# taleinat/fuzzysearch

Hardware: AMD Instinct MI355X
Metric: GB/s of sequence scanned at |p|=20 max_l_dist=2 (levenshtein_ngram path; two searches in flight: see value_sync for one synchronous call at a time) (higher is better)
Workload: dtype u8

## Files before the change

fuzzysearch_amd/_native.py:

```python
import ctypes
import os
import threading

_HERE = os.path.dirname(os.path.abspath(__file__))
LIB_PATH = os.environ.get("FUZZYSEARCH_HIP_LIB") or os.path.join(_HERE, "libfzhip.so")

FZ_OK, FZ_EINVAL, FZ_ENOMEM, FZ_EDEVICE, FZ_EUNSUPPORTED, FZ_EHALO, FZ_ETIMEOUT = 0, -1, -2, -3, -4, -5, -6
UINT64_MAX = (1 << 64) - 1


class FzMatch(ctypes.Structure):
    _fields_ = [("start", ctypes.c_int64), ("end", ctypes.c_int64),
                ("dist", ctypes.c_int32), ("block", ctypes.c_int32)]


class FzRecordsInfo(ctypes.Structure):
    _fields_ = [("n_lines", ctypes.c_uint64), ("n_seqs", ctypes.c_uint64), ("packed_bytes", ctypes.c_uint64),
                ("bad_record", ctypes.c_uint64), ("bad_reason", ctypes.c_uint32)]


class FzDeriveInfo(ctypes.Structure):
    _fields_ = [("n_out", ctypes.c_uint64), ("packed_bytes", ctypes.c_uint64), ("longest", ctypes.c_uint64),
                ("bad_item", ctypes.c_uint64), ("bad_reason", ctypes.c_uint32)]

# ... 60 lines not shown
    "fz_search_end": _END,
    "fz_subs_ngrams": _SEARCH,
    "fz_generic_ngrams": _GENERIC,
    "fz_generic_ngrams_consolidated": _GENERIC,
    "fz_lev_ngrams_consolidated": _SEARCH,
    "fz_subs_ngrams_best": _SEARCH,
    "fz_lev_ngrams_multi": _MULTI,
    "fz_lev_ngrams_multi_consolidated": _MULTI,
    "fz_debug_multi_plan": (ci, (bp, u64p, u32, u32, u32p, u32p)),
    "fz_subs_ngrams_multi": _MULTI,
    "fz_subs_ngrams_multi_best": _MULTI,
    "fz_debug_multi_plan_mode": (ci, (u32, bp, u64p, u32, u32, u32p, u32p)),
    "fz_batch_upload": (ci, (vp, bp, u64p, u64, vpp)),
    "fz_batch_search": (ci, (vp, vp, u32, bp, u32, u32, ci, mpp, u32pp, u64p)),
    "fz_batch_search_multi": (ci, (vp, vp, u32, bp, u64p, u32, u32, ci, mpp, u32pp, u64pp)),
    "fz_batch_assign": (ci, (vp, vp, u32, bp, u64p, u32, u32, vpp)),
    "fz_debug_assign_fold": (ci, (vp, u64, vp, u64, u32, vp, u32, vp, u32, u32, vp)),
    "fz_batch_end_overlaps": (ci, (vp, vp, u32, bp, u64p, u32, u32, u32, vpp)),
    "fz_debug_end_overlaps": (ci, (u32, bp, u64p, u32, u32, u32, bp, vp, u64, vp)),
    "fz_debug_overlap_ms": (ci, (vp, f64p)),
    "fz_batch_score_cuts": (ci, (vp, vp, vp, vp, u32, u32, u32, vpp)),
    "fz_debug_score_cuts": (ci, (vp, vp, u32, u32, u32, bp, vp, u64, vp)),
    "fz_debug_cuts_ms": (ci, (vp, f64p)),
    "fz_subs_ngrams_multi_cls": _MULTI_CLS,
    "fz_subs_ngrams_multi_best_cls": _MULTI_CLS,
    "fz_batch_search_multi_cls": (ci, (vp, vp, bp, u64p, u32, u32, bp, bp, ci, mpp, u32pp, u64pp)),
    "fz_batch_assign_cls": (ci, (vp, vp, bp, u64p, u32, u32, bp, bp, vpp)),
    "fz_debug_multi_plan_cls": (ci, (bp, u64p, u32, u32, bp, bp, u32p, u32p, u32p, u32p)),
    "fz_debug_batch_segment": (ci, (u64p, u64, u64, u64p, u64p, u64p)),
    "fz_batch_upload_records": (ci, (vp, bp, u64, u32, u32, u32, vpp, rip)),
    "fz_batch_tables": (ci, (vp, vp, vp)),
    "fz_debug_batch_bytes": (ci, (vp, vp, u64)),
    "fz_debug_records_split": (ci, (bp, u64, u32, u32, u32, vpp, vpp, vpp, rip)),
    "fz_debug_scan_items": (u32, ()),
    "fz_debug_records_ms": (ci, (vp, f64p)),
    "fz_batch_upload_fasta": (ci, (vp, bp, u64, u32, vpp, rip)),
    "fz_batch_fasta_index": (ci, (vp, vp)),
    "fz_debug_fasta_split": (ci, (bp, u64, u32, vpp, vpp, vpp, rip)),
    "fz_debug_fasta_upper4": (u32, (u32,)),
    "fz_debug_fasta_src": (u64, (u64, u64, u64, u64)),
    "fz_batch_derive": (ci, (vp, vp, vp, vp, vp, u64, u32, bp, vpp, dip)),
    "fz_debug_derive_plan": (ci, (vp, u64, vp, vp, vp, u64, vp, vp, dip)),
    "fz_debug_derive_ms": (ci, (vp, f64p)),
    "fz_batch_upload_records_lines": (ci, (vp, bp, u64, u32, vp, u32, u32, vpp, rip)),
    "fz_batch_format": (ci, (vp, vp, u32, bp, vp, u32, u32, vp, u64, fip)),
    "fz_debug_format_plan": (ci, (vp, u32, u64, vp, u32, u32, vp, fip)),
    "fz_debug_format_ms": (ci, (vp, f64p)),
    "fz_subs_ngrams_any": _ANY,
    "fz_subs_lp_any": _ANY,
    "fz_generic_ngrams_any": (ci, (vp, vp, bp, u32, u32, u32, u32, u32, cip)),
    "fz_lev_lp": _SEARCH,
    "fz_subs_lp": _SEARCH,
    "fz_generic_lp": _GENERIC,
    "fz_comm_unique_id": (ci, (vp, u64)),
    "fz_comm_init_rank": (ci, (vp, vp, ci, ci)),
    "fz_comm_init_all": (ci, (vp,)),
    "fz_comm_info": (ci, (vp, cip, cip, cip)),
    "fz_comm_set_collective": (ci, (vp, ci)),
    "fz_comm_allgather": (ci, (vp, vp, u64, vp)),
    "fz_comm_max_f64": (ci, (vp, f64p)),
    "fz_comm_barrier": (ci, (vp,)),
    "fz_comm_destroy": (None, (vp,)),
    "fz_comm_gather_ms": (ci, (vp, f64p)),
    "fz_comm_backend": (ci, ()),
    "fz_consolidate": _REDUCE,
    "fz_group_best": _REDUCE,
    "fz_merge_ranks": (ci, (vp, vp, vp, u32, u32, vp)),
    "fz_wire_pack": (ci, (vp, u64, u64, vp)),
    "fz_wire_merge": (ci, (vp, u32, u64, u64, vp, u64, u64p, u64p)),
    "fz_stream_open": (ci, (vp, u32, bp, u32, u32, u32, u32, u32, u64, u32, u32, u64, vpp)),
    "fz_stream_buffer": (ci, (vp, vpp, u64p)),
    "fz_stream_submit": (ci, (vp, u64, ci)),
    "fz_stream_read_fd": (ci, (vp, ci, i64, ci, u64p)),
    "fz_stream_finish": (ci, (vp, mpp, u32pp, u64p)),
    "fz_stream_close": (None, (vp,)),
    "fz_debug_reload_switches": (None, ()),
    "fz_debug_launch_plan": (ci, (bp, u32, u32, u32p, u32, u32p)),
    "fz_debug_order_records": (ci, (vp, u64, u32, mpp, u64p)),
    "fz_debug_order_records_bounded": (ci, (vp, u64, u32, u64, u32, mpp, u64p)),
    "fz_debug_order_segments": (ci, (vp, vp, u32, u32, mpp, u64p)),
    "fz_debug_scan_regions": (ci, (u64, u64, u32, ci, f64, ci, u32p, vp)),
    "fz_debug_scan_plan": (ci, (cs, u32, u32, u64, u32, ci, u32p, u32p, cip, u32p, vp)),
    "fz_debug_scan_instance": (ci, (u32, cs, u32, u32, u64, u32, u32p, u32p, u32p)),
    "fz_debug_gather_merge": (ci, (vp, u32, u64, vp, u32, mpp, u64p, u64p)),
    "fz_stats": (ci, (vp, stp)),
    "fz_mem_info": (ci, (vp, u64p, u64p)),
    "fz_set_timing": (ci, (vp, ci)),
    "fz_set_streams": (ci, (vp, ci)),
    "fz_device_ms": (ci, (vp, f64p, ci)),
    "fz_free": (None, (vp,)),
}
EXPORTED_SYMBOLS = tuple(PROTOTYPES)

OPTIONAL = frozenset((
    "fz_batch_search_multi", "fz_batch_assign", "fz_debug_assign_fold",
    "fz_batch_end_overlaps", "fz_debug_end_overlaps", "fz_debug_overlap_ms",
    "fz_batch_score_cuts", "fz_debug_score_cuts", "fz_debug_cuts_ms",
    "fz_subs_ngrams_multi_cls", "fz_subs_ngrams_multi_best_cls", "fz_batch_search_multi_cls", "fz_batch_assign_cls",
    "fz_debug_multi_plan_cls",
    "fz_batch_upload_records", "fz_batch_tables", "fz_debug_batch_bytes", "fz_debug_records_split", "fz_debug_scan_items",
    "fz_debug_records_ms",
    "fz_batch_upload_fasta", "fz_batch_fasta_index", "fz_debug_fasta_split", "fz_debug_fasta_upper4", "fz_debug_fasta_src",
    "fz_batch_derive", "fz_debug_derive_plan", "fz_debug_derive_ms",
    "fz_batch_upload_records_lines", "fz_batch_format", "fz_debug_format_plan", "fz_debug_format_ms",
    "fz_debug_scan_plan", "fz_mem_info", "fz_debug_scan_instance",
))

_lib = None
_lib_lock = threading.Lock()


def load_library():
    global _lib
    with _lib_lock:
        if _lib is not None:
            return _lib
        if not os.path.exists(LIB_PATH):
            raise HipEngineError(
                "fuzzysearch_amd: %s is missing. Build it with `python -m fuzzysearch_amd.build` "
                "(hipcc, --offload-arch=gfx950). There is no CPU fallback." % LIB_PATH)
        L = ctypes.CDLL(LIB_PATH)
        for name, (restype, argtypes) in PROTOTYPES.items():
            if name in OPTIONAL and not hasattr(L, name):
                continue
            fn = getattr(L, name)
            fn.restype, fn.argtypes = restype, argtypes
        if L.fz_abi_version() != 1:
            raise HipEngineError("libfzhip.so ABI version mismatch")
        _lib = L
        return L


class UnsupportedSearch(NotImplementedError):
    """The search is outside what the GPU engine supports: a subsequence of more than 65 535 items, a Levenshtein
    budget above 1 023, a generic search (separate limits) or a linear-programming route with max_l_dist above 255,
    more than 255 distinct symbols in a subsequence that is neither bytes nor latin-1 text, automaton candidate sets
    beyond 2^18 entries.  Nothing was searched and there is no CPU fallback: a caller that needs such a search
    catches this and routes it to the reference implementation."""


def _entry(lib, name):
    fn = getattr(lib, name, None)
    if fn is None:
        raise UnsupportedSearch("this libfzhip.so has no %s: it was built before that entry point existed" % name)
    return fn


def _raise(rc):
    msg = (load_library().fz_last_error() or b"").decode("utf-8", "replace")
    if rc == FZ_EINVAL:
        raise ValueError(msg)
    if rc == FZ_ENOMEM:
        raise MemoryError(msg)
    if rc == FZ_EUNSUPPORTED:
        raise UnsupportedSearch(msg)
    if rc == FZ_ETIMEOUT:
        raise CollectiveTimeout("libfzhip error %d: %s" % (rc, msg))
    raise HipEngineError("libfzhip error %d: %s" % (rc, msg))


def _check(rc):
    if rc != FZ_OK:
        _raise(rc)


def _buffer_address(data):
    mv = memoryview(data)
    if mv.itemsize != 1 or mv.ndim != 1 or not mv.c_contiguous:
        raise TypeError("only contiguous sequences of single-byte values are supported")
    n = mv.nbytes
    if n == 0:
        return None, 0, mv
    if mv.readonly:
        obj = mv.obj
        if isinstance(obj, bytes):
            return ctypes.cast(ctypes.c_char_p(obj), ctypes.c_void_p).value + _mv_offset(mv, obj), n, (mv, obj)
        import numpy as np
        arr = np.frombuffer(mv, dtype=np.uint8)
        return arr.ctypes.data, n, (mv, arr)
    c = (ctypes.c_char * n).from_buffer(mv)
    return ctypes.addressof(c), n, (mv, c)


def _mv_offset(mv, obj):
    if len(mv) == len(obj):
        return 0
    import numpy as np
    base = np.frombuffer(obj, dtype=np.uint8).ctypes.data
# ... 920 lines not shown
        ptr, bounds = self._multi_call(name, seq, patterns, k, tables)
        return OwnedRows(self._lib, ptr, bounds[-1]), bounds

    def subs_ngrams_multi_classes(self, seq, patterns, k, tables, best=False, as_array=False):
        return (self.subs_ngrams_multi_best if best else self.subs_ngrams_multi)(seq, patterns, k, as_array, tables)

    def multi_rows_call_classes(self, seq, patterns, k, tables):
        return self.multi_rows_call(seq, patterns, k, MODE_SUBS, tables)

    def lev_ngrams_begin(self, seq, pattern, k):
        paddr, m, keep = (pattern, len(pattern), None) if type(pattern) is bytes else _buffer_address(pattern)
        with self._lock:
            _check(self._lib.fz_lev_ngrams_begin(self._h, seq._h, paddr, m, k))

    def subs_ngrams_begin(self, seq, pattern, k):
        paddr, m, keep = (pattern, len(pattern), None) if type(pattern) is bytes else _buffer_address(pattern)
        with self._lock:
            _check(self._lib.fz_subs_ngrams_begin(self._h, seq._h, paddr, m, k))

    def generic_ngrams_begin(self, seq, pattern, max_subs, max_ins, max_dels, max_l, consolidated=False):
        paddr, m, keep = (pattern, len(pattern), None) if type(pattern) is bytes else _buffer_address(pattern)
        with self._lock:
            _check(self._lib.fz_generic_ngrams_begin(self._h, seq._h, paddr, m, max_subs, max_ins, max_dels, max_l,
                                                     1 if consolidated else 0))

    def search_end(self, as_array=False):
        return self.lev_ngrams_end(as_array=as_array)

    def lev_ngrams_end(self, as_array=False):
        ptr = mp()
        cnt = ctypes.c_uint64(0)
        with self._lock:
            _check(self._lib.fz_lev_ngrams_end(self._h, ctypes.byref(ptr), ctypes.byref(cnt)))
        if as_array:
            return _take_rows(self._lib, ptr, cnt.value)
        return _take_matches(self._lib, ptr, cnt.value)

    def subs_ngrams(self, seq, pattern, k, as_array=False):
        return self.rows_call(self._lib.fz_subs_ngrams, seq, pattern, k, take=_take_rows if as_array else _take_matches)

    def generic_ngrams(self, seq, pattern, max_subs, max_ins, max_dels, max_l, as_array=False):
        return self.rows_call(self._lib.fz_generic_ngrams, seq, pattern, max_subs, max_ins, max_dels, max_l,
                              take=_take_rows if as_array else _take_matches)

    def generic_ngrams_consolidated(self, seq, pattern, max_subs, max_ins, max_dels, max_l, as_array=False):
        return self.rows_call(self._lib.fz_generic_ngrams_consolidated, seq, pattern, max_subs, max_ins, max_dels, max_l,
                              take=_take_rows if as_array else _take_matches)

    def lev_lp(self, seq, pattern, k, as_array=False):
        return self.rows_call(self._lib.fz_lev_lp, seq, pattern, k, take=_take_rows if as_array else _take_matches)

    def subs_lp(self, seq, pattern, k, as_array=False):
        return self.rows_call(self._lib.fz_subs_lp, seq, pattern, k, take=_take_rows if as_array else _take_matches)

    def generic_lp(self, seq, pattern, max_subs, max_ins, max_dels, max_l, as_array=False):
        return self.rows_call(self._lib.fz_generic_lp, seq, pattern, max_subs, max_ins, max_dels, max_l,
                              take=_take_rows if as_array else _take_matches)

    def _any_call(self, fn, seq, pattern, *ints):
        paddr, m, keep = _buffer_address(pattern)
        found = ctypes.c_int(0)
        with self._lock:
            _check(fn(self._h, seq._h, paddr, m, *ints, ctypes.byref(found)))
        del keep
        return bool(found.value)

    def subs_ngrams_any(self, seq, pattern, k):
        return self._any_call(self._lib.fz_subs_ngrams_any, seq, pattern, k)

    def subs_lp_any(self, seq, pattern, k):
        return self._any_call(self._lib.fz_subs_lp_any, seq, pattern, k)

    def generic_ngrams_any(self, seq, pattern, max_subs, max_ins, max_dels, max_l):
        return self._any_call(self._lib.fz_generic_ngrams_any, seq, pattern, max_subs, max_ins, max_dels, max_l)

    def set_timing(self, on):
        with self._lock:
            _check(self._lib.fz_set_timing(self._h, 1 if on else 0))

    def set_streams(self, n):
        with self._lock:
            _check(self._lib.fz_set_streams(self._h, n))

    def stats(self):
        st = FzStats()
        with self._lock:
            _check(self._lib.fz_stats(self._h, ctypes.byref(st)))
        return {f: getattr(st, f) for f, _ in FzStats._fields_}

    def mem_info(self):
        f, t = ctypes.c_uint64(0), ctypes.c_uint64(0)
        with self._lock:
            _check(_entry(self._lib, 'fz_mem_info')(self._h, ctypes.byref(f), ctypes.byref(t)))
        return f.value, t.value

    def kernel_ms(self):
        with self._lock:
            st = self._st
            _check(self._lib.fz_stats(self._h, self._st_ref))
            return st.filter_ms, st.verify_ms, st.device_ms


_default_engine = None
_default_lock = threading.Lock()


def default_engine():
    global _default_engine
    with _default_lock:
        if _default_engine is None:
            env = os.environ.get("FUZZYSEARCH_HIP_DEVICES", "").strip()
            devices = [int(x) for x in env.split(",") if x.strip()] if env else None
            _default_engine = Engine(devices)
        return _default_engine
```

fuzzysearch_amd/csrc/fz_device.h:

```cpp
#pragma once
#include <stdint.h>

#if defined(__HIPCC__)
#define FZ_HD __host__ __device__ __forceinline__
#else
#define FZ_HD inline
#endif

#if defined(__HIP_DEVICE_COMPILE__)
#define FZ_WAVE_ANY(x) (__ballot((x) != 0) != 0ull)
#define FZ_WAVE_BALLOT(x) __ballot((x) != 0)
#else
#define FZ_WAVE_ANY(x) ((x) != 0)
#define FZ_WAVE_BALLOT(x) ((x) ? 1ull : 0ull)
#endif

#define FZ_MAX_BLOCKS_PER_LAUNCH 16
#define FZ_BLK_BITS 4
#define FZ_MAX_REGIONS 8
#define FZ_MAX_M 1024
#define FZ_MAX_K 255
#define FZ_MAX_M_ANY 65535u
#define FZ_MAX_K_ANY 1023u

// ... 65 lines not shown
    FzSeg r;
    r.sa = r.se = 0; r.j = 0; r.ok = 0;
    if (idx >= n || t.n_seqs == 0) return r;
    const uint64_t tile = idx >> FZ_RAG_TILE_BITS;
    uint32_t lo = t.first[tile], hi = t.first[tile + 1];
    if (hi >= t.n_seqs) hi = (uint32_t)t.n_seqs - 1u;
    while (lo < hi) {
        const uint32_t mid = lo + ((hi - lo) >> 1);
        if (t.ends[mid] > idx) hi = mid; else lo = mid + 1u;
    }
    r.sa = lo ? t.ends[lo - 1] : 0;
    r.se = t.ends[lo];
    r.j = lo;
    r.ok = 1;
    return r;
}

template <bool RAG>
FZ_HD uint32_t fz_segment_candidates_of(const FzGeom &g) { return RAG ? 1u : fz_segment_candidates(g); }
template <bool RAG>
FZ_HD FzSeg fz_segment_of(const FzGeom &g, uint64_t idx, uint32_t c) {
    if constexpr (RAG) {
        return fz_segment_ragged(fz_ragged(g), g.n, idx);
    } else {
        return fz_segment(g, idx, c);
    }
}

template <bool RAG>
FZ_HD FzSeg fz_segment_one(const FzGeom &g, uint64_t idx) {
    if constexpr (RAG) {
        return fz_segment_ragged(fz_ragged(g), g.n, idx);
    } else {
        FzSeg r;
        r.sa = 0; r.se = g.n; r.j = 0; r.ok = 1;
        return r;
    }
}

struct FzScanArgs {
    FzGeom   geom;
    uint32_t mode;
    uint32_t m, k;
    uint32_t L;
    uint32_t nblk;
    uint32_t g0;
    uint32_t d2;
    uint32_t mask1;
    uint32_t mask2;
    uint32_t fused;
    uint32_t band_w;
    uint32_t win_dwords;
    uint32_t vlanes;
    uint32_t max_subs, max_ins, max_dels;
    uint32_t cand_cap;
    uint64_t cand_scratch;
    uint32_t lp_kind;
    uint32_t lp_starts;
    uint32_t hash_k;
    uint32_t lut_shift;
    uint32_t gw;
    uint32_t qcap;
    uint32_t win_pieces;
    uint32_t flags;
    uint32_t H[FZ_MAX_BLOCKS_PER_LAUNCH];
    uint32_t A[FZ_MAX_BLOCKS_PER_LAUNCH];
    uint32_t B[FZ_MAX_BLOCKS_PER_LAUNCH];
    uint32_t lo_rel[FZ_MAX_BLOCKS_PER_LAUNCH];
    uint32_t hi_sub[FZ_MAX_BLOCKS_PER_LAUNCH];
    uint32_t s[FZ_MAX_BLOCKS_PER_LAUNCH];
    uint64_t abs_lo, abs_hi;
    uint64_t hit_cap;
    uint64_t rec_cap;
    uint64_t gen_order;
    uint64_t gen_dedup;
    uint64_t rows_cap;
    uint64_t host_hdr;
    uint64_t pat_g;
    uint8_t  pat[FZ_MAX_M];
    uint32_t nreg;
    uint32_t reg_wg0[FZ_MAX_REGIONS], reg_nwg[FZ_MAX_REGIONS];
    uint64_t reg_tile0[FZ_MAX_REGIONS], reg_end[FZ_MAX_REGIONS];
};

#define FZ_IDX_BITS 48
#define FZ_MAX_BLOCKS 65535u
struct FzRec {
    uint64_t key;
    uint32_t l;
    uint32_t r;
    uint32_t dist;
    uint32_t aux;
};

#define FZ_REC_NONE 0xffffffffu

FZ_HD uint64_t fz_hit_pack(uint32_t g, uint64_t idx) { return ((uint64_t)g << FZ_IDX_BITS) | idx; }
FZ_HD uint32_t fz_hit_block(uint64_t h) { return (uint32_t)(h >> FZ_IDX_BITS); }
FZ_HD uint64_t fz_hit_index(uint64_t h) { return h & ((1ull << FZ_IDX_BITS) - 1ull); }

FZ_HD uint32_t fz_hash_windows(uint32_t x, uint32_t yh, uint32_t k) { return (yh & 0xffffffu) * (k & 0xffffffu) + x; }
FZ_HD uint32_t fz_hash_short(uint32_t x_masked, uint32_t k) { return x_masked * k; }

template <class Sc, class SubF, class WinF>
FZ_HD bool fz_expand(Sc &sc, SubF sub, uint32_t sublen, WinF win, uint32_t winlen, uint32_t budget,
                     uint32_t &dist, uint32_t &consumed) {
    if (sublen == 0) { dist = 0; consumed = 0; return true; }
    const uint32_t big = budget + 1;
    const uint32_t W = 2 * budget + 2;
    uint32_t best = sublen, arg = 0;
    {
        uint32_t rows = budget < sublen ? budget : sublen;
        for (uint32_t i = 1; i <= rows; ++i) sc.set(i, i);
    }
    uint32_t jmax = winlen;
    if (jmax > sublen + budget) jmax = sublen + budget;
    uint32_t i0 = 1, slot0 = 1;
    for (uint32_t j = 1; j <= jmax; ++j) {
        const uint8_t ch = win(j - 1);
        if (j > budget + 1) { ++i0; slot0 = (slot0 + 1 == W) ? 0 : slot0 + 1; }
        uint32_t i1 = j + budget; if (i1 > sublen) i1 = sublen;
        if (i0 > i1) break;
        uint32_t a, c;
        if (i0 == 1) { a = j - 1; c = j; }
        else { a = sc.get(slot0 == 0 ? W - 1 : slot0 - 1); c = big; }
        uint32_t slot = slot0;
        uint32_t cmin = c;
        for (uint32_t i = i0; i <= i1; ++i) {
            uint32_t b = (i + 1 > j + budget) ? big : sc.get(slot);
            uint32_t v = a + (ch != sub(i - 1) ? 1u : 0u);
            if (b + 1 < v) v = b + 1;
            if (c + 1 < v) v = c + 1;
            sc.set(slot, v);
            c = v;
            a = b;
            if (v < cmin) cmin = v;
            slot = (slot + 1 == W) ? 0 : slot + 1;
        }
        if (i1 == sublen && c <= best) { best = c; arg = j; }
        if (cmin > budget) break;
    }
    if (best <= budget) { dist = best; consumed = arg; return true; }
    return false;
}

#define FZ_REG_BAND_MAX 8
template <int K, class SubF, class WinF>
FZ_HD bool fz_expand_band(SubF sub, uint32_t sublen, WinF win, uint32_t winlen, uint32_t budget,
                          uint32_t &dist, uint32_t &consumed) {
    if (sublen == 0) { dist = 0; consumed = 0; return true; }
    constexpr uint32_t INF = 0x3fffffffu;
    constexpr int W = 2 * K + 1;
    uint32_t cell[W];
    uint32_t chr[W];
#pragma unroll
    for (int x = 0; x < W; ++x) {
        const int d = x - K;
        cell[x] = (d >= 0 && (uint32_t)d <= winlen) ? (uint32_t)d : INF;
        chr[x] = (d >= 0 && (uint32_t)d < winlen) ? (uint32_t)win((uint32_t)d) : 0x100u;
    }
    for (uint32_t i = 1; i <= sublen; ++i) {
        const uint32_t pc = sub(i - 1);
        uint32_t left = INF, rowmin = INF;
#pragma unroll
        for (int x = 0; x < W; ++x) {
            const int d = x - K;
// ... 1394 lines not shown
```

fuzzysearch_amd/csrc/fz_kernel_bodies.inc:

```
#if FZ_KERNEL_BODY == 1
    constexpr bool WF = WFG == 16 || WFG == 32;
    constexpr int BITS = (WFG == 1 || WFG == 2 || WFG == 4) ? WFG : 0;
    constexpr bool ADAPT = BITS != 0 || WFG == 3;
    constexpr int VF = WFG == 3 ? -1 : BITS;
    static_assert(WFG == 0 || ADAPT || WF, "0: register band / Hamming count; 3: Hamming count; 1, 2, 4: bit-vector columns; 16, 32: lanes per candidate");
    static_assert(!(SEG && RAG), "strided and ragged segments are two geometries");
    static_assert(WFG == 0 || (FUSED && !SEG), "the lane-per-cell and bit-vector forms are fused forms of the in-memory search");
    constexpr bool PREF = FUSED && !SEG && !WF;
    constexpr uint32_t peq_bytes = BITS ? FZ_PEQ_BYTES(BITS ? BITS : 1) : 0u;
    extern __shared__ __attribute__((aligned(16))) uint8_t smem[];
    const uint32_t mpad = FUSED ? (a.m + 15u) & ~15u : 0u;
    uint32_t *lut = reinterpret_cast<uint32_t *>(smem);
    if (reinterpret_cast<uintptr_t>((FzLdsU8 *)smem) != 0) __builtin_trap();
    uint8_t *pat_lds = smem + FZ_TABLE_BYTES;
    if constexpr (FUSED)
        for (uint32_t i = threadIdx.x; i < a.m; i += FZ_FILTER_THREADS) pat_lds[i] = a.pat[i];
    if constexpr (BITS != 0) {
        constexpr int NWc = BITS ? BITS : 1;
        uint32_t *peq = reinterpret_cast<uint32_t *>(smem + FZ_TABLE_BYTES + mpad);
        constexpr uint32_t wdw = FZ_BITS_WIDTH(NWc) / 32u;
        for (uint32_t i = threadIdx.x; i < peq_bytes / 4u; i += FZ_FILTER_THREADS) peq[i] = 0u;
        __syncthreads();
        if (threadIdx.x < a.m) {
            const uint32_t q = threadIdx.x, c = pat_lds[q];
            const uint32_t bf = fz_bits_fwd_bit<NWc>(a.m, q), br = fz_bits_rev_bit<NWc>(a.m, q);
            atomicOr(&peq[c * wdw + (bf >> 5)], 1u << (bf & 31u));
            atomicOr(&peq[(256u + c) * wdw + (br >> 5)], 1u << (br & 31u));
        }
    }
    if (threadIdx.x < FZ_LUT_SLOTS) {
        uint32_t t = ((threadIdx.x + 1u) & (FZ_LUT_SLOTS - 1u)) << a.lut_shift;
        uint32_t who = 0xffu;
        uint32_t set = 0;
        for (uint32_t g = a.nblk; g-- > 0;)
            if (((a.H[g] >> a.lut_shift) & (FZ_LUT_SLOTS - 1u)) == threadIdx.x) { t = a.H[g]; who = g; set |= 0x10000u << g; }
        lut[threadIdx.x] = t;
        if constexpr (DUPH) lut[FZ_LUT_SLOTS + threadIdx.x] = (a.flags & FZ_FLAG_DUP_HASHES) ? (who | set) : who;
        else lut[FZ_LUT_SLOTS + threadIdx.x] = who;
    }
    bool dup_hashes = false;
    if constexpr (DUPH) dup_hashes = (a.flags & FZ_FLAG_DUP_HASHES) != 0;
    uint32_t wg0 = 0, stride = gridDim.x;
    uint64_t tile0 = 0, limit = ntiles;
#pragma unroll
    for (uint32_t r = 0; r < FZ_MAX_REGIONS; ++r)
        if (r < a.nreg && blockIdx.x >= a.reg_wg0[r]) { wg0 = a.reg_wg0[r]; stride = a.reg_nwg[r]; tile0 = a.reg_tile0[r]; limit = a.reg_end[r]; }
    const uint64_t first_tile = tile0 + (blockIdx.x - wg0);
    if (threadIdx.x == 0) {
        uint32_t *walk = reinterpret_cast<uint32_t *>(smem + FZ_WALK_LDS);
        walk[0] = (uint32_t)first_tile; walk[1] = (uint32_t)(first_tile >> 32); walk[2] = stride;
    }
    __syncthreads();
    const uint32_t wave = (uint32_t)__builtin_amdgcn_readfirstlane((int)(threadIdx.x >> 6));
    const uint32_t qcap = PREF ? a.qcap : (uint32_t)FZ_QCAP;
    const FzWaveLds w = PREF ? fz_wave_lds_pref(smem + FZ_TABLE_BYTES + mpad + peq_bytes, FZ_TABLE_BYTES + mpad + peq_bytes, wave, qcap, a.win_pieces)
                        : WF ? fz_wave_lds(smem + FZ_TABLE_BYTES + mpad, wave, fz_wf_fused_dwords(a.win_dwords, WF ? WFG : 16), 0u, 1u, true)
                             : fz_wave_lds(smem + FZ_TABLE_BYTES + mpad, wave, FUSED ? a.win_dwords : 0u,
                                           FUSED ? a.band_w : 0u, a.vlanes, true);
    const uint32_t hash_k = a.hash_k;
    uint32_t slot_shift;
    asm volatile("v_mov_b32 %0, %1" : "=v"(slot_shift) : "s"(a.lut_shift - 2u));
    const uint32_t mask1 = a.mask1;
    const uint32_t lane = fz_lane();
    const uint32_t lane_off = threadIdx.x * 16u;
    uint32_t qn = 0;
    uint32_t qf = 0;
    uint32_t confirmed = 0;
    uint32_t titer = 0;
    uint64_t tile = first_tile;
    if ((a.flags & FZ_FLAG_ANY) && __hip_atomic_load(&counters[1], __ATOMIC_RELAXED, __HIP_MEMORY_SCOPE_AGENT) != 0ull) tile = limit;
    bool slow = false;
    uint32_t slow_pos = 0;
    uint32_t ylast = 0;
    uint32_t b0 = 0, bw = FZ_MAX_BLOCKS_PER_LAUNCH;

    auto test_row = [&](const uint4 &v, const uint2 &h, auto Rc) {
        constexpr int r = decltype(Rc)::value;
        constexpr int GRP = FZ_GROUP ? FZ_GROUP : (NWIN == 2 && DH == 5 && !FUSED ? 8 : 4);
        const uint32_t w6[6] = {v.x, v.y, v.z, v.w, h.x, h.y};
#pragma unroll
        for (int j = 0; j < 16 / GRP; ++j) {
            uint32_t hv[GRP], lv[GRP];
#pragma unroll
            for (int i = 0; i < GRP; ++i) {
                const int o = GRP * j + i;
                const uint32_t x = FZ_WIN(w6, o);
                if (NWIN == 1) hv[i] = (x & mask1) * hash_k;
                else hv[i] = __umul24(FZ_WIN(w6, o + DH), hash_k) + x;
                uint32_t slot4;
                if constexpr (SA) asm("v_and_b32 %0, " FZ_LUT_ADDR_MASK_STR ", %1" : "=v"(slot4) : "v"(hv[i]));
                else asm("v_lshrrev_b32 %0, %1, %2\n\tv_and_b32 %0, " FZ_LUT_ADDR_MASK_STR ", %0" : "=v"(slot4) : "v"(slot_shift), "v"(hv[i]));
                lv[i] = *reinterpret_cast<FzLdsU32 *>(slot4);
            }
            uint32_t am[GRP];
#pragma unroll
            for (int i = 0; i < GRP; ++i) am[i] = hv[i] ^ lv[i];
            uint32_t acc = min(min(am[0], am[1]), min(am[2], am[3]));
            if constexpr (GRP == 8) acc = min(acc, min(min(am[4], am[5]), min(am[6], am[7])));
            const bool fire = __ballot(acc == 0) != 0;
            if (__builtin_expect(fire, 0)) {
#pragma unroll
                for (int i = 0; i < GRP; ++i) {
                    const unsigned long long mi = __ballot(hv[i] == lv[i]);
                    if (mi) {
                        uint32_t slot4;
                        if constexpr (SA) asm("v_and_b32 %0, " FZ_LUT_ADDR_MASK_STR ", %1" : "=v"(slot4) : "v"(hv[i]));
                        else asm("v_lshrrev_b32 %0, %1, %2\n\tv_and_b32 %0, " FZ_LUT_ADDR_MASK_STR ", %0" : "=v"(slot4) : "v"(slot_shift), "v"(hv[i]));
                        const uint32_t g = *reinterpret_cast<FzLdsU32 *>(slot4 + FZ_LUT_BYTES);
                        uint32_t pos = threadIdx.x;
                        asm volatile("v_lshlrev_b32 %0, 4, %0" : "+v"(pos));
                        if (DUPH && __builtin_expect(dup_hashes, 0)) {
                            uint32_t set = hv[i] == lv[i] ? g >> 16 : 0u;
                            pos += (uint32_t)(r * FZ_ROW_BYTES + GRP * j + i);
                            while (__ballot(set != 0u)) {
                                const uint32_t gb = (uint32_t)__ffs((int)set) - 1u;
                                const bool take = set != 0u && (!ADAPT || gb - b0 < bw);
                                const unsigned long long mk = __ballot(take);
                                const uint32_t slot = qn + fz_rank(mk);
                                if (take && slot < qcap) w.queue[slot] = fz_code(pos, gb, titer);
                                qn += (uint32_t)__popcll(mk);
                                set &= set - 1u;
                            }
                        } else if constexpr (ADAPT) {
                            const bool take = hv[i] == lv[i] && g - b0 < bw;
                            const unsigned long long mt = __ballot(take);
                            const uint32_t slot = qn + fz_rank(mt);
                            if (take && slot < qcap)
                                w.queue[slot] = fz_code(pos + (uint32_t)(r * FZ_ROW_BYTES + GRP * j + i), g, titer);
                            qn += (uint32_t)__popcll(mt);
                        } else {
                            const uint32_t slot = qn + fz_rank(mi);
                            if (hv[i] == lv[i] && slot < qcap)
                                w.queue[slot] = fz_code(pos + (uint32_t)(r * FZ_ROW_BYTES + GRP * j + i), g, titer);
                            qn += (uint32_t)__popcll(mi);
                        }
                    }
                }
            }
        }
    };

    for (;;) {
        if (slow) {
            const uint32_t nb = ADAPT ? min(bw, a.nblk - b0) : a.nblk;
            const uint32_t steps = FZ_FILTER_ROWS * 16u * nb;
            while (slow_pos < steps && qn + 64u <= qcap) {
                const uint32_t blk = (ADAPT ? b0 : 0u) + slow_pos % nb;
                const uint32_t ro = slow_pos / nb;
                w.queue[qn + lane] = fz_code((ro >> 4) * FZ_ROW_BYTES + lane_off + (ro & 15u), blk, titer);
                qn += 64u;
                ++slow_pos;
            }
            if (slow_pos >= steps) {
                slow = false;
                if (ADAPT && b0 + bw < a.nblk) b0 += bw;
                else { b0 = 0; tile += stride; ++titer; }
            }
        } else if (tile < limit && (ADAPT ? (qn == 0u || qn + ylast + (ylast >> 2) + 8u <= qcap) : qn <= qcap / 2)) {
            uint4 va[2], vb[2];
            uint2 ha[2], hb[2];
            bool pre;
            {
                const uint8_t *tsrc = buf + fz_bcast64(tile * (uint64_t)FZ_TILE_BYTES);
#pragma unroll
                for (int r = 0; r < 2; ++r) {
                    va[r] = *reinterpret_cast<const uint4 *>(tsrc + r * FZ_ROW_BYTES + lane_off);
                    ha[r] = *reinterpret_cast<const uint2 *>(tsrc + r * FZ_ROW_BYTES + lane_off + 16);
                }
            }
            do {
                const uint8_t *tsrc = buf + fz_bcast64(tile * (uint64_t)FZ_TILE_BYTES);
#pragma unroll
                for (int r = 0; r < 2; ++r) {
                    vb[r] = *reinterpret_cast<const uint4 *>(tsrc + (r + 2) * FZ_ROW_BYTES + lane_off);
                    hb[r] = *reinterpret_cast<const uint2 *>(tsrc + (r + 2) * FZ_ROW_BYTES + lane_off + 16);
                }
                __builtin_amdgcn_sched_barrier(0);
                const uint32_t q_tile = qn;
                test_row(va[0], ha[0], std::integral_constant<int, 0>{});
                test_row(va[1], ha[1], std::integral_constant<int, 1>{});
                const bool same_tile = ADAPT && b0 + bw < a.nblk;
                const uint64_t next = same_tile ? tile : tile + stride;
                if constexpr (ADAPT) pre = next < limit && qn + 3u * (qn - q_tile) + 8u <= qcap;
                else pre = next < limit && qn <= qcap / 2;
                {
                    const uint8_t *nsrc = buf + fz_bcast64((pre ? next : tile) * (uint64_t)FZ_TILE_BYTES);
#pragma unroll
                    for (int r = 0; r < 2; ++r) {
                        va[r] = *reinterpret_cast<const uint4 *>(nsrc + r * FZ_ROW_BYTES + lane_off);
                        ha[r] = *reinterpret_cast<const uint2 *>(nsrc + r * FZ_ROW_BYTES + lane_off + 16);
                    }
                }
                __builtin_amdgcn_sched_barrier(0);
                test_row(vb[0], hb[0], std::integral_constant<int, 2>{});
                test_row(vb[1], hb[1], std::integral_constant<int, 3>{});
                if (qn > qcap) {
                    qn = q_tile;
                    if constexpr (ADAPT) {
                        if (q_tile != 0u) {
                            ylast = qcap;
                            break;
                        }
                        const uint32_t nb = min(bw, a.nblk - b0);
                        if (nb > 1u) {
                            bw = (nb + 1u) >> 1;
                            ylast = qcap >> 1;
                            break;
                        }
                    }
                    slow = true;
                    slow_pos = 0;
                    break;
                }
                if constexpr (ADAPT) ylast = qn - q_tile;
                if (PREF && qn > qf) {
                    if (tile) fz_prefetch_tile(buf, a, w, qf, qn, tile * (uint64_t)FZ_TILE_BYTES);
                    else fz_prefetch_windows(buf, a, w, qf, qn);
                    qf = qn;
                }
                if constexpr (ADAPT) {
                    if (same_tile) {
                        b0 += bw;
                    } else {
                        b0 = 0;
                        if (bw < a.nblk && ylast <= (qcap >> 3)) bw <<= 1;
                        tile = next;
                        ++titer;
                    }
                } else {
                    tile = next;
                    ++titer;
                }
            } while (pre);
        }
        const bool done = !slow && tile >= limit;
        if (PREF && done) break;
        if constexpr (WF) {
            confirmed += fz_flush_wf<WF ? WFG : 16, RAG>(buf, a, smem, pat_lds, w, smem + FZ_TABLE_BYTES + mpad,
                                                    fz_wave_lds_bytes(fz_wf_fused_dwords(a.win_dwords, WF ? WFG : 16), 0u, 1u, true),
                                                    reinterpret_cast<volatile uint32_t *>(smem + 2u * FZ_LUT_BYTES), wave, qn, done, recs, counters);
        } else if (qn) {
            if (PREF && qn > qf) fz_prefetch_windows(buf, a, w, qf, qn);
            if constexpr (ADAPT) {
                confirmed += fz_bits_flush<VF, RAG>(buf, a, pat_lds, smem + FZ_TABLE_BYTES + mpad, w, qn, recs, counters);
                qf = qn;
                continue;
            } else {
                confirmed += fz_queue_flush<FUSED, SEG, RAG, MAXK>(buf, a, pat_lds, w, qn, hits, recs, counters);
            }
        }
        qn = 0;
        qf = 0;
        if (done) break;
    }
    if constexpr (PREF) {
        if (qn > qf) fz_prefetch_windows(buf, a, w, qf, qn);
        confirmed += fz_pooled_flush<MAXK, VF, RAG>(buf, a, pat_lds, smem + FZ_TABLE_BYTES + mpad + peq_bytes, fz_wave_lds_pref_bytes(qcap, a.win_pieces),
                                              reinterpret_cast<volatile uint32_t *>(smem + 2u * FZ_LUT_BYTES), wave, qn, recs, counters,
                                              smem + FZ_TABLE_BYTES + mpad);
    }

    if (FUSED && lane == 0 && confirmed) atomicAdd(&counters[8 + (blockIdx.x & 63u)], (unsigned long long)confirmed);
    fz_finish_launch(a, counters, lut);
#elif FZ_KERNEL_BODY == 2
    extern __shared__ __attribute__((aligned(16))) uint8_t smem[];
    const uint32_t mpad = (a.m + 15u) & ~15u;
    uint8_t *pat_lds = smem;
    fz_copy_pattern(pat_lds, a, threadIdx.x, blockDim.x);
    __syncthreads();
    const FzWaveLds w = fz_wave_lds(smem + mpad, threadIdx.x >> 6, a.win_dwords, a.band_w, a.vlanes, false);
    unsigned long long nh = counters[0];
    if (nh > a.hit_cap) nh = a.hit_cap;
    const uint64_t waves = (uint64_t)gridDim.x * (blockDim.x >> 6);
    const uint64_t wave = (uint64_t)blockIdx.x * (blockDim.x >> 6) + (threadIdx.x >> 6);
    const uint32_t ncand = fz_segment_candidates_of<RAG>(a.geom);
    for (uint64_t q0 = wave * a.vlanes; q0 < nh; q0 += waves * a.vlanes) {
        const uint64_t q = q0 + fz_lane();
        const bool have = fz_lane() < a.vlanes && q < nh;
        const uint64_t hit = have ? hits[q] : 0;
        for (uint32_t c = 0; c < ncand; ++c) {
            const FzSeg sg = fz_segment_of<RAG>(a.geom, fz_hit_index(hit), c);
            const bool valid = have && fz_hit_in_range_s(a, fz_hit_block(hit) * a.L, fz_hit_index(hit), sg);
            if (!__ballot(valid)) continue;
            fz_wave_verify<FZ_REG_BAND_MAX, false>(buf, a, pat_lds, w, fz_lane(), hit, sg, valid, recs, counters);
        }
    }
    fz_finish_launch(a, counters, reinterpret_cast<uint32_t *>(smem));
#elif FZ_KERNEL_BODY == 3
    extern __shared__ __attribute__((aligned(16))) uint8_t smem[];
    constexpr uint32_t NH = 64u / (uint32_t)GW;
    const uint32_t mpad = (a.m + 15u) & ~15u;
    uint8_t *pat_lds = smem + 16;
    fz_copy_pattern(pat_lds, a, threadIdx.x, blockDim.x);
    __syncthreads();
    const uint32_t lane = fz_lane();
    const uint32_t grp = lane / (uint32_t)GW, gl = lane % (uint32_t)GW;
    const uint32_t wbytes = a.win_dwords * 4u;
    uint8_t *gwin = smem + 16 + mpad + 16 + ((threadIdx.x >> 6) * NH + grp) * (wbytes + 16u);
    unsigned long long nh = counters[0];
    if (nh > a.hit_cap) nh = a.hit_cap;
    const uint64_t waves = (uint64_t)gridDim.x * (blockDim.x >> 6);
    const uint64_t wave = (uint64_t)blockIdx.x * (blockDim.x >> 6) + (threadIdx.x >> 6);
    const uint32_t ncand = fz_segment_candidates_of<RAG>(a.geom);
    const uint64_t per_wg = (uint64_t)NH * (blockDim.x >> 6);
    uint32_t active_wgs = (uint32_t)((nh + per_wg - 1) / per_wg < gridDim.x ? (nh + per_wg - 1) / per_wg : gridDim.x);
    if (active_wgs == 0) active_wgs = 1;
    if (blockIdx.x >= active_wgs) return;
    const bool compact = nh * ncand > FZ_WF_COMPACT_MIN;
    for (uint64_t q0 = wave * NH; q0 < nh; q0 += waves * NH) {
        const uint64_t q = q0 + grp;
        const bool have = q < nh;
        const uint64_t hit = have ? hits[q] : 0;
        const uint32_t g = fz_hit_block(hit);
        const uint64_t idx = fz_hit_index(hit);
        const uint32_t s = g * a.L;
        for (uint32_t c = 0; c < ncand; ++c) {
            const FzSeg sg = fz_segment_of<RAG>(a.geom, idx, c);
            const bool valid = have && fz_hit_in_range_s(a, s, idx, sg);
// ... 406 lines not shown
```

fuzzysearch_amd/csrc/fz_kernels.h:

```cpp
#pragma once
#include <hip/hip_runtime.h>
#include <cstddef>
#include <type_traits>
#include "fz_device.h"

#define FZ_FILTER_THREADS 256
#define FZ_WAVES_PER_BLOCK (FZ_FILTER_THREADS / 64)
#define FZ_FILTER_ROWS 4
#define FZ_ROW_BYTES (FZ_FILTER_THREADS * 16)
#define FZ_TILE_BYTES (FZ_ROW_BYTES * FZ_FILTER_ROWS)
#define FZ_TILE_BITS 14
#define FZ_TITER_MAX ((1u << (32 - FZ_TILE_BITS - FZ_BLK_BITS)) - 1)
#define FZ_PAD_FRONT 256
#define FZ_PAD_BACK 256
#ifndef FZ_GROUP
#define FZ_GROUP 0
#endif
#define FZ_WF_COMPACT_MIN 8192ull
#define FZ_QCAP 256
#ifndef FZ_LUT_BITS
#define FZ_LUT_BITS 5
#endif
#define FZ_LUT_SLOTS (1u << FZ_LUT_BITS)
#define FZ_LUT_BYTES (FZ_LUT_SLOTS * 4u)
#define FZ_TABLE_BYTES (2u * FZ_LUT_BYTES + 32u)
#define FZ_WALK_LDS (2u * FZ_LUT_BYTES + 16u)
#define FZ_FLAG_DUP_HASHES 1u
#define FZ_FLAG_FOLD 4u
#define FZ_FLAG_ANY 2u
#if FZ_LUT_BITS == 5
#define FZ_LUT_ADDR_MASK_STR "0x7c"
#else
#define FZ_LUT_ADDR_MASK_STR "0xfc"
#endif

__device__ __forceinline__ uint32_t fz_win(uint32_t lo, uint32_t hi, int b) {
    return b == 0 ? lo : __builtin_amdgcn_alignbyte(hi, lo, (uint32_t)b);
}
#define FZ_WIN(w, o) fz_win((w)[(o) >> 2], (w)[((o) >> 2) + 1], (o) & 3)

typedef __attribute__((address_space(3))) const uint32_t FzLdsU32;
typedef __attribute__((address_space(3))) uint8_t FzLdsU8;

__device__ __forceinline__ uint32_t fz_lane() { return threadIdx.x & 63u; }

__device__ __forceinline__ void fz_copy_pattern(uint8_t *dst, const FzScanArgs &a, uint32_t tid, uint32_t nthreads) {
    if (a.pat_g) {
        const uint8_t *pg = reinterpret_cast<const uint8_t *>(a.pat_g);
        for (uint32_t i = tid; i < a.m; i += nthreads) dst[i] = pg[i];
    } else {
        for (uint32_t i = tid; i < a.m; i += nthreads) dst[i] = a.pat[i];
    }
}

__device__ __forceinline__ uint32_t fz_rank(unsigned long long mask) {
    return __builtin_amdgcn_mbcnt_hi((uint32_t)(mask >> 32), __builtin_amdgcn_mbcnt_lo((uint32_t)mask, 0u));
}

__device__ __forceinline__ void fz_wave_lds_sync() {
    __builtin_amdgcn_fence(__ATOMIC_RELEASE, "workgroup");
    __builtin_amdgcn_wave_barrier();
    __builtin_amdgcn_fence(__ATOMIC_ACQUIRE, "workgroup");
}

__device__ __forceinline__ uint32_t fz_load_win(const uint8_t *__restrict__ buf, int64_t local) {
    const int64_t base = local & ~(int64_t)3;
    const uint32_t lo = *reinterpret_cast<const uint32_t *>(buf + base);
    const uint32_t hi = *reinterpret_cast<const uint32_t *>(buf + base + 4);
    return __builtin_amdgcn_alignbyte(hi, lo, (uint32_t)(local & 3));
}


struct FzWaveLds {
    uint32_t *queue;
    uint32_t *win;
    uint16_t *scores;
    uint32_t win_lds;
};

__host__ __device__ inline uint32_t fz_wave_lds_bytes(uint32_t win_dwords, uint32_t band_w, uint32_t vlanes,
                                                      bool with_queue) {
    uint32_t b = 0;
    if (with_queue) b += FZ_QCAP * 4;
    b += win_dwords * vlanes * 4;
    b += ((band_w * vlanes * 2) + 15u) & ~15u;
    return b;
}

__host__ __device__ inline uint32_t fz_wf_fused_dwords(uint32_t win_dwords, uint32_t gw) { return (64u / gw) * (win_dwords + 4u); }

__device__ __forceinline__ FzWaveLds fz_wave_lds(uint8_t *base, uint32_t wave, uint32_t win_dwords, uint32_t band_w,
                                                 uint32_t vlanes, bool with_queue) {
    uint8_t *p = base + (size_t)wave * fz_wave_lds_bytes(win_dwords, band_w, vlanes, with_queue);
    FzWaveLds w;
    w.queue = nullptr;
    if (with_queue) { w.queue = reinterpret_cast<uint32_t *>(p); p += FZ_QCAP * 4; }
    w.win = reinterpret_cast<uint32_t *>(p); p += win_dwords * vlanes * 4;
    w.scores = reinterpret_cast<uint16_t *>(p);
    w.win_lds = 0;
    return w;
}

__host__ __device__ inline uint32_t fz_wave_lds_pref_bytes(uint32_t qcap, uint32_t win_pieces) {
    return qcap * 4u + win_pieces * qcap * 16u;
}

__device__ __forceinline__ FzWaveLds fz_wave_lds_pref(uint8_t *base, uint32_t base_lds, uint32_t wave, uint32_t qcap,
                                                      uint32_t win_pieces) {
    const uint32_t off = wave * fz_wave_lds_pref_bytes(qcap, win_pieces);
    FzWaveLds w;
    w.queue = reinterpret_cast<uint32_t *>(base + off);
    w.win = reinterpret_cast<uint32_t *>(base + off + qcap * 4u);
// ... 160 lines not shown
            FzLdsScores sc{w.scores + (PREF ? 0u : vl), a.vlanes};
            if (valid) ok = fz_verify_lev<MAXK>(sc, t, sg.sa, sg.se, pat_lds, a.m, a.k, a.L, s, idx, rec);
        } else if (valid) {
            ok = fz_verify_subs(t, pat_lds, a.m, a.k, a.L, s, idx, rec);
        }
        return confirmed;
    };
    uint32_t confirmed;
    if constexpr (PREF) {
        confirmed = run(FzDmaWindow{pref_win, wbase, a.qcap * 16u});
    } else {
        confirmed = run(FzLdsWindow{reinterpret_cast<const uint8_t *>(w.win + vl), wbase, a.vlanes * 4u});
    }
    const unsigned long long mask = __ballot(ok);
    if (mask) {
        unsigned long long base = 0;
        if (lane == 0) base = atomicAdd(&counters[1], (unsigned long long)__popcll(mask));
        base = fz_bcast64(base);
        if (ok) {
            rec.key = hit;
            rec.aux = sg.j;
            const unsigned long long slot = base + fz_rank(mask);
            if (slot < a.rec_cap) recs[slot] = rec;
        }
    }
    fz_wave_lds_sync();
    return confirmed;
}

__device__ __forceinline__ bool fz_confirm(const uint8_t *__restrict__ buf, const FzScanArgs &a, uint32_t blk,
                                           uint64_t local) {
    if ((fz_load_win(buf, (int64_t)local) & a.mask1) != a.A[blk]) return false;
    if (a.L > 4 && (fz_load_win(buf, (int64_t)local + a.d2) & a.mask2) != a.B[blk]) return false;
    if (a.L > 8) {
        if (a.pat_g) {
            const uint8_t *pg = reinterpret_cast<const uint8_t *>(a.pat_g) + a.s[blk];
            for (uint32_t b = 8; b < a.L; ++b)
                if (buf[local + b] != pg[b]) return false;
        } else {
            for (uint32_t b = 8; b < a.L; ++b)
                if (buf[local + b] != a.pat[a.s[blk] + b]) return false;
        }
    }
    return true;
}

#define FZ_HDR_WORDS 128
#define FZ_HDR_TICKET 3
#define FZ_HDR_SHARD0 96
#define FZ_TICKET_SHARDS 16u

__device__ __forceinline__ void fz_finish_launch(const FzScanArgs &a, unsigned long long *__restrict__ counters,
                                                 volatile uint32_t *flag, uint32_t participants = 0) {
    if (!a.host_hdr) return;
    if (participants == 0) participants = gridDim.x;
    __syncthreads();
    if (threadIdx.x == 0) {
        const uint32_t nshard = participants < FZ_TICKET_SHARDS ? participants : FZ_TICKET_SHARDS;
        const uint32_t r = blockIdx.x % nshard;
        const unsigned long long members = (participants - r + nshard - 1u) / nshard;
        bool last = atomicAdd(&counters[FZ_HDR_SHARD0 + r], 1ull) == members - 1ull;
        if (last) last = atomicAdd(&counters[FZ_HDR_TICKET], 1ull) == (unsigned long long)nshard - 1ull;
        *flag = last ? 1u : 0u;
    }
    __syncthreads();
    if (*flag) {
        unsigned long long *dst = reinterpret_cast<unsigned long long *>(a.host_hdr);
        for (uint32_t i = threadIdx.x; i < FZ_HDR_WORDS; i += blockDim.x) {
            dst[i] = __hip_atomic_load(&counters[i], __ATOMIC_RELAXED, __HIP_MEMORY_SCOPE_AGENT);
            __hip_atomic_store(&counters[i], 0ull, __ATOMIC_RELAXED, __HIP_MEMORY_SCOPE_AGENT);
        }
    }
}

__device__ __forceinline__ uint32_t fz_uniform(uint32_t v) { return (uint32_t)__builtin_amdgcn_readfirstlane((int)v); }

__device__ __forceinline__ uint32_t fz_code(uint32_t off, uint32_t blk, uint32_t titer) {
    return off | (blk << FZ_TILE_BITS) | (titer << (FZ_TILE_BITS + FZ_BLK_BITS));
}

__device__ __forceinline__ uint64_t fz_code_local(uint32_t code, uint32_t &blk) {
    blk = (code >> FZ_TILE_BITS) & (FZ_MAX_BLOCKS_PER_LAUNCH - 1u);
    FzLdsU32 *walk = (FzLdsU32 *)(uintptr_t)FZ_WALK_LDS;
    const uint64_t first = ((uint64_t)walk[1] << 32) | walk[0];
    const uint64_t tile = first + (uint64_t)(code >> (FZ_TILE_BITS + FZ_BLK_BITS)) * walk[2];
    return tile * (uint64_t)FZ_TILE_BYTES + (code & (FZ_TILE_BYTES - 1u));
}

__device__ __forceinline__ void fz_prefetch_windows(const uint8_t *__restrict__ buf, const FzScanArgs &a,
                                                    const FzWaveLds &w, uint32_t qf, uint32_t qn) {
    const uint32_t lane = fz_lane();
    asm volatile("" ::: "memory");
    for (uint32_t e0 = qf; e0 < qn; e0 += 64u) {
        const uint32_t e = e0 + lane;
        if (e < qn) {
            uint32_t blk;
            const uint64_t idx = a.geom.buf_off + fz_code_local(w.queue[e], blk);
            const uint64_t wbase = fz_window_base(a, fz_window_lo(a, idx, (a.g0 + blk) * a.L, 0));
            const uint8_t *src = buf + (wbase - a.geom.buf_off);
            for (uint32_t c = 0; c < a.win_pieces; ++c)
                fz_glds16(src + 16u * c, (uint32_t)__builtin_amdgcn_readfirstlane((int)(w.win_lds + (c * a.qcap + e0) * 16u)));
        }
    }
}

__device__ __forceinline__ void fz_prefetch_tile(const uint8_t *__restrict__ buf, const FzScanArgs &a, const FzWaveLds &w,
                                                 uint32_t qf, uint32_t qn, uint64_t tile_local) {
    const uint32_t lane = fz_lane();
    asm volatile("" ::: "memory");
    constexpr uint32_t BIAS = 2048u;
    const uint8_t *sbase = buf + fz_bcast64(tile_local) - BIAS;
    const uint32_t c0 = a.g0 * a.L + a.k;
    for (uint32_t e0 = qf; e0 < qn; e0 += 64u) {
        const uint32_t e = e0 + lane;
        if (e < qn) {
            const uint32_t code = w.queue[e];
            const uint32_t reach = ((code >> FZ_TILE_BITS) & (FZ_MAX_BLOCKS_PER_LAUNCH - 1u)) * a.L + c0;
            const uint32_t voff = (((code & (FZ_TILE_BYTES - 1u)) - reach) & ~3u) + BIAS;
            for (uint32_t c = 0; c < a.win_pieces; ++c) {
                const uint32_t lds_dst = fz_uniform(w.win_lds + (c * a.qcap + e0) * 16u);
                uint32_t keep;
                asm volatile("s_mov_b32 %0, m0\n\ts_mov_b32 m0, %3\n\ts_nop 0\n\tglobal_load_lds_dwordx4 %1, %2\n\ts_mov_b32 m0, %0"
                             : "=&s"(keep) : "v"(voff + 16u * c), "s"(sbase), "s"(lds_dst) : "memory");
            }
        }
    }
}

__device__ __forceinline__ void fz_gen_claim(const FzScanArgs &a, uint64_t hit, unsigned long long q) {
    if (q >= FZ_GEN_ORDER_MAX) return;
    const FzGenDedup dd(a.gen_dedup);
    const uint32_t blk = fz_hit_block(hit);
    const unsigned long long wk = fz_hit_index(hit) + a.k - (unsigned long long)blk * a.L + 1ull;
    uint32_t slot = (uint32_t)((wk * 0x9E3779B97F4A7C15ull) >> 40) & (FZ_GEN_DEDUP_SLOTS - 1u);
    uint32_t at = FZ_GEN_DEDUP_NONE;
    for (uint32_t probe = 0; probe < 32u; ++probe) {
        const unsigned long long old = atomicCAS(&dd.keys[slot], 0ull, wk);
        if (old == 0ull || old == wk) { at = slot; break; }
        slot = (slot + 1u) & (FZ_GEN_DEDUP_SLOTS - 1u);
    }
    if (at != FZ_GEN_DEDUP_NONE) {
        const uint32_t pos = atomicAdd(&dd.nmem[at], 1u);
        if (pos < FZ_GEN_DEDUP_MEMBERS) dd.mem[at * FZ_GEN_DEDUP_MEMBERS + pos] = (uint32_t)q;
        else at = FZ_GEN_DEDUP_NONE;
    }
    if (at != FZ_GEN_DEDUP_NONE) atomicMax(&dd.best[at], ~(((unsigned long long)blk << 32) | q));
    dd.wslot[q] = at;
}

template <int GW, bool RAG>
__device__ __forceinline__ uint32_t fz_flush_wf(const uint8_t *__restrict__ buf, const FzScanArgs &a, const uint8_t *lds0,
                                                const uint8_t *pat_lds, const FzWaveLds &w, const uint8_t *area, uint32_t per_wave,
                                                volatile uint32_t *fills, uint32_t wave, uint32_t qn, bool pooled,
                                                FzRec *__restrict__ recs, unsigned long long *__restrict__ counters);

template <bool FUSED, bool SEG, bool RAG, int MAXK = 4>
__device__ __forceinline__ uint32_t fz_queue_flush(const uint8_t *__restrict__ buf, const FzScanArgs &a,
                                                   const uint8_t *pat_lds, const FzWaveLds &w, uint32_t qn,
                                                   uint64_t *__restrict__ hits, FzRec *__restrict__ recs,
                                                   unsigned long long *__restrict__ counters) {
    constexpr bool PREF = FUSED && !SEG;
    const uint32_t lane = fz_lane();
    uint32_t confirmed = 0;
    if (PREF) asm volatile("s_waitcnt vmcnt(0)" ::: "memory");
    fz_wave_lds_sync();
    const uint32_t width = (FUSED && !PREF) ? a.vlanes : 64u;
    const uint32_t ncand = (SEG && FUSED) ? fz_segment_candidates(a.geom) : 1u;
    for (uint32_t e0 = 0; e0 < qn; e0 += width) {
        for (uint32_t c = 0; c < ncand; ++c) {
// ... 2023 lines not shown
```

fuzzysearch_amd/csrc/fzhip.hip:

```cpp
#include <hip/hip_runtime.h>
#include <hip/hip_ext.h>
#include <rccl/rccl.h>
#include <dlfcn.h>

#include <algorithm>
#include <atomic>
#include <chrono>
#include <condition_variable>
#include <cstdarg>
#include <cstdio>
#include <cstdlib>
#include <cstring>
#include <functional>
#include <new>
#include <string>
#include <thread>
#include <unistd.h>
#include <map>
#include <mutex>
#include <vector>
#include <cassert>

#include "../../include/fzhip.h"
#include "fz_kernels.h"

namespace {

struct Switches {
    bool no_direct = false;
    bool no_slot_and = false;
    int max_blocks = 0;
    bool force_big_verify = false;
    bool no_wf_fuse = false;
    int wf32 = -1;
    bool no_bits = false;
    int bits_min_k = 3;
    int bits_qcap = 0;
    bool gen_legacy = false;
    bool gen_no_dedup = false;
    int gh_waves = 0;
    bool gh_no_bits = false;
    int cand_lds_max = 0;
    bool mp_force_pass = false;
    bool no_dev_threads = false;
    int taper_steps = 4;
    double taper_min = 0.25;
    int taper_wg_per_cu = 7;
    bool no_rccl = false;
    std::string rccl_lib;
    std::string rocm_path = "/opt/rocm";
    long comm_timeout_ms = 60000;
    bool trace = false;
    bool stream_trace = false;
};

Switches read_switches() {
        Switches v;
        auto flag = [](const char *n) { return getenv(n) != nullptr; };
        auto num = [](const char *n, int dflt) { const char *e = getenv(n); return e ? atoi(e) : dflt; };
        v.no_direct = flag("FZ_NO_DIRECT"); v.no_slot_and = flag("FZ_NO_SLOT_AND"); v.max_blocks = num("FZ_MAX_BLOCKS", 0);
        v.force_big_verify = flag("FZ_FORCE_BIG_VERIFY"); v.no_wf_fuse = flag("FZ_NO_WF_FUSE");
        v.no_bits = flag("FZ_NO_BITS"); v.bits_min_k = num("FZ_BITS_MIN_K", 3); v.bits_qcap = num("FZ_BITS_QCAP", 0);
        v.wf32 = num("FZ_WF32", -1); v.gen_legacy = flag("FZ_GEN_LEGACY"); v.gen_no_dedup = flag("FZ_GEN_NO_DEDUP");
        v.gh_waves = num("FZ_GH_WAVES", 0); v.gh_no_bits = flag("FZ_GH_NO_BITS"); v.cand_lds_max = num("FZ_CAND_LDS_MAX", 0);
        v.no_dev_threads = flag("FZ_NO_DEV_THREADS"); v.taper_steps = num("FZ_TAPER_STEPS", 4);
        if (const char *e = getenv("FZ_TAPER_MIN")) v.taper_min = atof(e);
        v.taper_wg_per_cu = num("FZ_TAPER_WG_PER_CU", 7); v.no_rccl = flag("FZ_NO_RCCL");
        if (const char *e = getenv("FZ_RCCL_LIB")) v.rccl_lib = e;
        if (const char *e = getenv("ROCM_PATH")) v.rocm_path = e;
        if (const char *e = getenv("FZ_COMM_TIMEOUT_MS")) v.comm_timeout_ms = std::max(1L, atol(e));
        v.mp_force_pass = flag("FZ_MP_FORCE_PASS");
        v.trace = flag("FZ_TRACE"); v.stream_trace = flag("FZ_STREAM_TRACE");
        return v;
}

Switches &switches_storage() { static Switches s = read_switches(); return s; }
const Switches &sw() { return switches_storage(); }

struct Trace {
    bool on;
    std::chrono::steady_clock::time_point t0, last;
    Trace() : on(sw().trace) { t0 = last = std::chrono::steady_clock::now(); }
    void mark(const char *what) {
        if (!on) return;
        auto now = std::chrono::steady_clock::now();
        fprintf(stderr, "[fz] %-18s %8.1f us (total %8.1f)\n", what,
                std::chrono::duration<double, std::micro>(now - last).count(),
                std::chrono::duration<double, std::micro>(now - t0).count());
        last = now;
    }
};

thread_local std::string g_err;

bool env_no_direct() { return sw().no_direct; }

int fail(int code, const char *fmt, ...) {
    char tmp[512];
    va_list ap;
    va_start(ap, fmt);
    vsnprintf(tmp, sizeof tmp, fmt, ap);
    va_end(ap);
    g_err = tmp;
    return code;
}

#define HIP_TRY(expr)                                                                              \
    do {                                                                                           \
        hipError_t e_ = (expr);                                                                    \
        if (e_ != hipSuccess)                                                                      \
            return fail(e_ == hipErrorOutOfMemory ? FZ_ENOMEM : FZ_EDEVICE, "%s failed: %s", #expr, \
                        hipGetErrorString(e_));                                                    \
    } while (0)

constexpr uint64_t kHeaderBytes = 1024;
constexpr uint64_t kFirstCopyRecs = 4096;
constexpr uint64_t kHostRecs = 16384;
static_assert(kHeaderBytes == FZ_HDR_WORDS * 8, "header layout");

struct SearchRun {
    bool last_direct = false;
    bool timed = true;
    bool fused_used = false;
    uint32_t form_used = 0;
    uint32_t launches_used = 0;
    bool verify_launched = false;
    int scan_end_event = 1;
    int verify_end_event = 2;
    bool on_alt = false;
    uint64_t hit_cap_used = 0, rec_cap_used = 0;
    bool dedup_used = false;
    bool gen_multi_used = false;
    bool fold_was_direct = false;
    uint64_t fold_copied = 0;
    int lp_end_event = 2;
};

struct ResultSlot {
    hipEvent_t ev[4] = {nullptr, nullptr, nullptr, nullptr};
    uint8_t *h_stage = nullptr;
    uint8_t *h_stage_dev = nullptr;
    uint8_t *d_send = nullptr;
    hipEvent_t ev_snap = nullptr;
    bool snap_taken = false;
    SearchRun run;
};

struct DevState {
    int device = 0;
    hipStream_t stream = nullptr;
    ResultSlot slots[2];
    int slot_id = 0;
    ResultSlot &cur() { return slots[slot_id]; }
    const ResultSlot &cur() const { return slots[slot_id]; }
    void swap_slot() { slot_id ^= 1; }
    uint64_t *d_hits = nullptr;
    uint64_t hit_cap = 0;
    uint8_t *d_out = nullptr;
    uint64_t rec_cap = 0;
    bool direct = true;
    uint8_t *d_cand = nullptr;
    uint64_t cand_bytes = 0;
    uint8_t *d_gen_order = nullptr;
    uint8_t *d_gen_rows = nullptr;
    uint8_t *d_gen_dedup = nullptr;
    bool dedup_zeroed = false;
    uint64_t gen_dedup_arg = 0;
    uint64_t gen_rows_cap = 0;
    uint8_t *h_big = nullptr;
    uint64_t big_cap = 0;
    uint8_t *spare_alloc = nullptr;
    uint64_t spare_bytes = 0;
    hipEvent_t rec_ev[10] = {};
    uint64_t first_copy = 512;
    bool header_zeroed = false;
    uint8_t *stream_h[2] = {nullptr, nullptr};
    uint8_t *stream_d = nullptr;
    uint64_t stream_cap = 0, stream_d_bytes = 0;
    int n_cus = 256;
    double last_filter_ms = 0;
    uint64_t fold_guess = 8192;
    bool fold_direct = true;
    uint8_t *d_pat = nullptr;
    uint64_t pat_cap = 0;
    uint8_t *d_mp_desc = nullptr, *d_mp_ctr = nullptr, *d_mp_hits = nullptr, *d_mp_recs = nullptr;
    uint64_t mp_hit_cap = 0, mp_rec_cap = 0;
    uint32_t mp_desc_words = 0;
    uint8_t *d_assign = nullptr, *d_assign_recs = nullptr;
    uint64_t assign_cap = 0, assign_rec_cap = 0;
    hipStream_t stream_alt = nullptr;
    uint8_t *d_hdr_alt = nullptr;
    ncclComm_t comm = nullptr;
    int comm_rank = -1;
    hipStream_t comm_stream = nullptr;
    uint64_t send_cap = 0;
    uint8_t *d_recv = nullptr, *h_recv = nullptr;
    uint64_t recv_bytes = 0;
    hipEvent_t ev_done = nullptr;
};

struct TimingRef { DevState *d; hipEvent_t f0, f1, v0, v1, t0, t1; };
TimingRef timing_ref(DevState &d, bool generic) {
    const ResultSlot &s = d.cur();
    hipEvent_t v0 = generic || s.run.verify_launched ? s.ev[1] : nullptr;
    return {&d, s.ev[0], s.ev[s.run.scan_end_event], v0, s.ev[generic ? s.run.lp_end_event : s.run.verify_end_event], s.ev[0], s.ev[3]};
}

inline bool geom_is_ragged(const FzGeom &g) { return g.seg_stride == 0 && g.seg_j1 != 0; }

struct Shard {
    int dev = 0;
    uint8_t *d_alloc = nullptr;
    uint8_t *d_buf = nullptr;
    uint64_t alloc_bytes = 0;
    FzGeom geom{};
};

}

namespace {

struct DevWorkers {
    struct W {
        std::thread th;
        std::mutex mu;
        std::condition_variable cv;
        std::function<int()> job;
        std::atomic<uint64_t> posted{0}, done{0};
        int rc = 0;
        std::string err;
        bool stop = false;
    };
    std::vector<W *> ws;
    static constexpr long kSpinUs = 1500;

    explicit DevWorkers(size_t n) {
        for (size_t i = 0; i < n; ++i) {
            W *w = new W();
            ws.push_back(w);
            w->th = std::thread([this, w]() { run(w); });
        }
    }
    ~DevWorkers() {
        for (W *w : ws) {
            { std::lock_guard<std::mutex> g(w->mu); w->stop = true; }
            w->cv.notify_one();
            w->th.join();
            delete w;
        }
    }
    void run(W *w) {
        uint64_t seen = 0;
        for (;;) {
            const auto t0 = std::chrono::steady_clock::now();
            unsigned spins = 0;
            while (w->posted.load(std::memory_order_acquire) == seen) {
                if ((++spins & 255u) == 0 &&
                    std::chrono::duration_cast<std::chrono::microseconds>(std::chrono::steady_clock::now() - t0).count() > kSpinUs) {
                    std::unique_lock<std::mutex> lk(w->mu);
                    w->cv.wait(lk, [&]() { return w->stop || w->posted.load(std::memory_order_acquire) != seen; });
                    if (w->stop) return;
                    break;
                }
                __builtin_ia32_pause();
            }
            seen = w->posted.load(std::memory_order_acquire);
            try {
                w->rc = w->job();
                if (w->rc) w->err = g_err;
            } catch (const std::bad_alloc &) {
                w->rc = FZ_ENOMEM; w->err = "out of memory on a device worker thread";
            } catch (const std::exception &e) {
                w->rc = FZ_EDEVICE; w->err = std::string("exception on a device worker thread: ") + e.what();
            }
            w->done.store(seen, std::memory_order_release);
        }
    }
    void post(size_t i, std::function<int()> fn) {
        W *w = ws[i];
        while (w->done.load(std::memory_order_acquire) != w->posted.load(std::memory_order_relaxed)) std::this_thread::yield();
        w->job = std::move(fn);
        w->posted.fetch_add(1, std::memory_order_release);
        { std::lock_guard<std::mutex> g(w->mu); }
        w->cv.notify_one();
    }
    int wait(size_t i) {
        W *w = ws[i];
        const uint64_t want = w->posted.load(std::memory_order_relaxed);
        unsigned spins = 0;
        while (w->done.load(std::memory_order_acquire) != want) {
            if ((++spins & 1023u) == 0) std::this_thread::yield(); else __builtin_ia32_pause();
        }
        if (w->rc) g_err = w->err;
        return w->rc;
    }
};

struct ShardOut {
    std::vector<FzRec> recs;
    std::vector<uint64_t> hits;
    std::vector<fz_match> rows;
    bool rerun = false;
    uint64_t nh = 0, nr = 0, bytes = 0;
    TimingRef tref{};
};

}

struct fz_ctx {
    std::vector<DevState> devs;
    fz_stats_t stats{};
    uint32_t gen_cand_cap = 256;
    bool gen_multi = !sw().gen_legacy;
    uint32_t gen_multi_skip = 0, gen_multi_backoff = 0;
    const FzRec *view = nullptr;
    uint64_t view_n = 0;
    const FzGenRec *gen_view = nullptr;
    uint64_t gen_view_n = 0;
    const uint8_t *gen_rows_dev = nullptr;
    uint64_t gen_rows_n = 0;
    int gen_rows_device = 0;
    struct fz_stream *stream_inflight = nullptr;
    struct Pending {
        fz_seq *seq = nullptr;
        std::vector<uint8_t> pattern;
        uint32_t m = 0, k = 0;
        bool launched = false;
        uint32_t kind = FZ_MODE_LEV;
        uint32_t max_subs = 0, max_ins = 0, max_dels = 0;
        bool consolidated = false;
        int lane = 0;
    } pend[2];
    int npend = 0;
    std::vector<DevState> devs2;
    int lane = 0;
    std::vector<fz_seq *> live;
    bool any_found = false;
    double rec_ms[4] = {0, 0, 0, 0};
    double drv_ms[5] = {0, 0, 0, 0, 0};
    double fmt_ms[5] = {0, 0, 0, 0, 0};
    double ovl_ms[4] = {0, 0, 0, 0};
    double cut_ms[4] = {0, 0, 0, 0};
    bool batch_call = false;
    std::vector<size_t> seg_ends;
    std::vector<uint32_t> seg_order;
    bool timing = true;
    std::vector<TimingRef> tref;
    int comm_world = 0;
    bool snapshot = false;
    bool comm_broken = false;
    uint64_t gcap = 4096;
    int streams = 1;
    double last_gather_ms = 0;
    DevWorkers *workers = nullptr;
    std::vector<ShardOut> souts;
    bool rows_ready = false;
};

struct fz_seq {
    fz_ctx *ctx = nullptr;
    uint64_t n = 0;
    std::vector<Shard> shards;
    std::vector<uint64_t> rank_lo;
    bool is_batch = false;
    uint64_t n_seqs = 0;
    std::vector<uint64_t> ends;
    uint64_t *d_ends_base = nullptr;
    uint32_t *d_first = nullptr;
    uint64_t max_seq_len = 0;
    uint64_t *d_src_starts = nullptr;
    FzFaRow *d_fa_rows = nullptr;
    bool is_fasta = false;
};

namespace {
void comm_teardown(fz_ctx *ctx);
inline DevState &lane_dev(fz_ctx *ctx, int dev) { return ctx->lane ? ctx->devs2[dev] : ctx->devs[dev]; }

void resolve_timing(fz_ctx *ctx) {
    for (const TimingRef &r : ctx->tref) {
        float f = 0, v = 0, t = 0;
        if (hipSetDevice(r.d->device) != hipSuccess) continue;
        if (r.f0 && hipEventElapsedTime(&f, r.f0, r.f1) != hipSuccess) f = 0;
        if (r.v0 && hipEventElapsedTime(&v, r.v0, r.v1) != hipSuccess) v = 0;
        if (r.t0 && hipEventElapsedTime(&t, r.t0, r.t1) != hipSuccess) t = 0;
        (void)hipGetLastError();
        r.d->last_filter_ms = f;
        ctx->stats.filter_ms = std::max<double>(ctx->stats.filter_ms, f);
        ctx->stats.verify_ms = std::max<double>(ctx->stats.verify_ms, v);
        ctx->stats.device_ms = std::max<double>(ctx->stats.device_ms, t);
    }
    ctx->tref.clear();
}
}

namespace {

template <class T>
int grow_device(DevState &d, T *&ptr, uint64_t &have, uint64_t cap, uint64_t bytes) {
    if (have >= cap) return FZ_OK;
    HIP_TRY(hipSetDevice(d.device));
    if (ptr) { HIP_TRY(hipFree(ptr)); ptr = nullptr; have = 0; }
    HIP_TRY(hipMalloc(reinterpret_cast<void **>(&ptr), (size_t)bytes));
    have = cap;
    return FZ_OK;
}

double span_ms(hipEvent_t a, hipEvent_t b) {
    float ms = 0;
    if (hipEventElapsedTime(&ms, a, b) != hipSuccess) ms = 0;
    (void)hipGetLastError();
    return (double)ms;
}

int ensure_hits(DevState &d, uint64_t cap) { return grow_device(d, d.d_hits, d.hit_cap, cap, cap * sizeof(uint64_t)); }

constexpr uint32_t kCandLdsMax = 4096;
constexpr uint32_t kCandMax = 1u << 18;
constexpr unsigned kCandScratchGrid = 256;

int cand_lists(DevState &d, uint32_t cand_cap, size_t fixed_lds, size_t &lds, uint64_t &scratch) {
    if (fixed_lds > 150 * 1024) return fail(FZ_EUNSUPPORTED, "subsequence + window too long for the automaton kernel's LDS (%zu bytes)", fixed_lds);
    lds = fixed_lds + 2 * (size_t)cand_cap * sizeof(FzGCand);
    scratch = 0;
    const uint32_t lds_max = sw().cand_lds_max > 0 ? (uint32_t)sw().cand_lds_max : kCandLdsMax;
    if (cand_cap <= lds_max && lds <= 160 * 1024) return FZ_OK;
    if (cand_cap > kCandMax) return fail(FZ_EUNSUPPORTED, "automaton candidate sets beyond %u entries", kCandMax);
    lds = fixed_lds;
    const uint64_t need = (uint64_t)kCandScratchGrid * 2 * cand_cap * sizeof(FzGCand);
    int rc = grow_device(d, d.d_cand, d.cand_bytes, need, need);
    if (rc) return rc;
    scratch = reinterpret_cast<uint64_t>(d.d_cand);
    return FZ_OK;
}

// ... 248 lines not shown
    fa.abs_hi = q.plan.abs_hi;
    if (q.m <= FZ_MAX_M) memcpy(fa.pat, q.p, q.m);
}


int stage_pattern(DevState &d, FzScanArgs &fa, const uint8_t *p, uint32_t m, bool force = false) {
    fa.pat_g = 0;
    if (m <= FZ_MAX_M && !force) return FZ_OK;
    HIP_TRY(hipSetDevice(d.device));
    if (d.pat_cap < m) {
        HIP_TRY(hipStreamSynchronize(d.stream));
        const uint64_t cap = std::max<uint64_t>(4096, (uint64_t)m * 2);
        int rc = grow_device(d, d.d_pat, d.pat_cap, cap, cap);
        if (rc) return rc;
    }
    HIP_TRY(hipMemcpyAsync(d.d_pat, p, m, hipMemcpyHostToDevice, d.stream));
    fa.pat_g = reinterpret_cast<uint64_t>(d.d_pat);
    return FZ_OK;
}

int wavefront_group(uint32_t k) { return 2 * k + 1 <= 16 ? 16 : 2 * k + 1 <= 32 ? 32 : 64; }

struct VerifyPlan {
    bool want_wf = false, big = false;
    int gw = 16;
    size_t wf_lds = 0, ring_lds = 0;
    unsigned waves = 4;
};

VerifyPlan plan_verify(const Search &q) {
    const bool force_big = sw().force_big_verify;
    VerifyPlan v;
    const uint32_t mpad = (q.m + 15u) & ~15u;
    const uint32_t win_dwords = (q.m + 2 * q.k + 6) / 4 + 1;
    const uint32_t band_w = q.mode == FZ_MODE_LEV ? 2 * q.k + 2 : 0;
    v.gw = wavefront_group(q.k);
    const uint32_t wf_per_wave = (64u / v.gw) * (win_dwords * 4u + 16u);
    v.wf_lds = 16 + mpad + 16 + 16 * (size_t)wf_per_wave;
    while (v.waves > 1 && mpad + v.waves * (size_t)fz_wave_lds_bytes(win_dwords, band_w, 64, false) > 64 * 1024) v.waves >>= 1;
    v.ring_lds = mpad + (size_t)v.waves * fz_wave_lds_bytes(win_dwords, band_w, 64, false);
    v.want_wf = q.mode == FZ_MODE_LEV && q.k >= 5 && q.k <= 31;
    v.big = force_big || q.m > FZ_MAX_M || q.k > FZ_MAX_K || (v.want_wf ? v.wf_lds > 64 * 1024 : v.ring_lds > 160 * 1024);
    return v;
}

void plan_scan_regions(FzScanArgs &fa, uint64_t ntiles, uint64_t grid, uint32_t n_cus, int steps, double fmin, int t_per_cu) {
    fa.nreg = 0;
    steps = std::min(steps, FZ_MAX_REGIONS - 1);
    fmin = std::min(1.0, std::max(0.02, fmin));
    const uint64_t Gw = grid, T = (uint64_t)n_cus * (uint64_t)std::max(1, t_per_cu);
    if (steps <= 0 || (uint64_t)steps > T || Gw < 2 * T || ntiles < 4 * Gw) return;
    const uint64_t per = T / steps;
    double weight = (double)(Gw - T);
    std::vector<double> f(steps);
    std::vector<uint64_t> nw(steps);
    for (int j = 0; j < steps; ++j) {
        f[j] = 1.0 - (1.0 - fmin) * (j + 1) / steps;
        nw[j] = j + 1 < steps ? per : T - per * (steps - 1);
        weight += f[j] * (double)nw[j];
    }
    const double share = (double)ntiles / weight;
    uint64_t at = 0, wg = 0;
    auto add = [&](uint64_t nwg, uint64_t tiles) {
        fa.reg_wg0[fa.nreg] = (uint32_t)wg; fa.reg_nwg[fa.nreg] = (uint32_t)nwg;
        fa.reg_tile0[fa.nreg] = at; fa.reg_end[fa.nreg] = at + tiles;
        ++fa.nreg; wg += nwg; at += tiles;
    };
    add(Gw - T, std::min<uint64_t>(ntiles, (uint64_t)(share * (double)(Gw - T) + 0.5)));
    for (int j = 0; j < steps; ++j) {
        const uint64_t left = ntiles - at;
        add(nw[j], j + 1 < steps ? std::min<uint64_t>(left, (uint64_t)(share * f[j] * (double)nw[j] + 0.5)) : left);
    }
    for (uint32_t r = 0; r < fa.nreg; ++r)
        if ((fa.reg_end[r] - fa.reg_tile0[r] + fa.reg_nwg[r] - 1) / fa.reg_nwg[r] >= FZ_TITER_MAX) { fa.nreg = 0; break; }
}

void plan_scan_regions(FzScanArgs &fa, uint64_t ntiles, uint64_t grid, uint32_t n_cus) {
    const int steps = sw().taper_steps;
    const double fmin = sw().taper_min;
    const int t_per_cu = sw().taper_wg_per_cu;
    plan_scan_regions(fa, ntiles, grid, n_cus, steps, fmin, t_per_cu);
}

struct ScanPlan {
    uint64_t ntiles = 0;
    uint32_t grid = 1;
    int wfg = 0;
    uint32_t form = FZ_FORM_NONE;
    uint32_t lds = 0;
    VerifyPlan vp;
    bool overlapped = false;
};

ScanPlan plan_scan(const Search &q, const FzGeom &geom, uint32_t n_cus, bool with_verify, bool shares_chip, FzScanArgs &fa) {
    ScanPlan sp;
    const uint32_t L = q.plan.L;
    const uint32_t G = (uint32_t)q.plan.s.size();
    const bool in_memory = geom.seg_stride == 0;
    const uint64_t ntiles_all = (geom.buf_len + FZ_TILE_BYTES - 1) / FZ_TILE_BYTES;
    const uint64_t tile_lo = std::min<uint64_t>(ntiles_all, q.part_lo / FZ_TILE_BYTES);
    const uint64_t tile_hi = q.part_hi == ~0ull ? ntiles_all : std::min<uint64_t>(ntiles_all, (q.part_hi + FZ_TILE_BYTES - 1) / FZ_TILE_BYTES);
    const bool partial = tile_lo != 0 || tile_hi != ntiles_all;
    const uint64_t ntiles = sp.ntiles = tile_hi > tile_lo ? tile_hi - tile_lo : 0;
    const bool force_big = sw().force_big_verify;
    sp.vp = plan_verify(q);
    const VerifyPlan &vp = sp.vp;
    fa.band_w = q.mode == FZ_MODE_LEV ? 2 * q.k + 2 : 0;
    fa.win_dwords = (q.m + 2 * q.k + 6) / 4 + 1;
    const uint32_t mpad = (q.m + 15u) & ~15u;
    constexpr uint32_t target = 18u * 1024u;
    fa.vlanes = 64;
    uint32_t fused_lds;
    if (in_memory) {
        fa.win_pieces = (q.m + 2 * q.k + 3 + 15) / 16;
        fa.qcap = 128;
        while (fa.qcap > 64 && mpad + FZ_TABLE_BYTES + FZ_WAVES_PER_BLOCK * fz_wave_lds_pref_bytes(fa.qcap, fa.win_pieces) > target + 4096)
            fa.qcap >>= 1;
        fused_lds = mpad + FZ_TABLE_BYTES + FZ_WAVES_PER_BLOCK * fz_wave_lds_pref_bytes(fa.qcap, fa.win_pieces);
        if (fa.win_pieces * 16u + 16u > FZ_PAD_BACK) fused_lds = ~0u;
    } else {
        while (fa.vlanes > 16 && mpad + FZ_TABLE_BYTES + FZ_WAVES_PER_BLOCK * fz_wave_lds_bytes(fa.win_dwords, fa.band_w, fa.vlanes, true) > target)
            fa.vlanes >>= 1;
        fused_lds = mpad + FZ_TABLE_BYTES + FZ_WAVES_PER_BLOCK * fz_wave_lds_bytes(fa.win_dwords, fa.band_w, fa.vlanes, true);
    }
    fa.fused = (with_verify && !force_big && q.m <= FZ_MAX_M && q.k <= FZ_MAX_K && fused_lds <= kFusedLdsBudget &&
                (q.mode != FZ_MODE_LEV || q.k <= 4)) ? 1u : 0u;
    int bits_nw = 0;
    double per_tile = 0;
    {
        bool seen[256] = {false};
        uint32_t sigma = 0;
        for (uint32_t i = 0; i < q.m; ++i)
            if (!seen[q.p[i]]) { seen[q.p[i]] = true; ++sigma; }
        per_tile = 4096.0 * std::min<uint32_t>(G, FZ_MAX_BLOCKS_PER_LAUNCH);
        for (uint32_t i = 0; i < L && per_tile > 0.01; ++i) per_tile /= (double)std::max(2u, sigma);
    }
    const bool bits_budget = q.k >= (uint32_t)sw().bits_min_k || per_tile > 16.0;
    static_assert(FZ_PAD_BACK - 16 <= 255, "fz_verify_lev_bits: window columns in 8 bits");
    if (q.mode == FZ_MODE_LEV && with_verify && !force_big && !sw().no_bits && in_memory && bits_budget &&
        q.m <= FZ_BITS_MAX_M(2) && q.k <= FZ_MAX_K && fa.win_pieces * 16u + 16u <= FZ_PAD_BACK) {
        bits_nw = q.m <= FZ_BITS_MAX_M(4) ? 4 : q.m <= FZ_BITS_MAX_M(1) ? 1 : 2;
        constexpr uint32_t budget = 26u * 1024u;
        const uint32_t fixed = mpad + FZ_TABLE_BYTES + FZ_PEQ_BYTES(bits_nw);
        uint32_t qc = sw().bits_qcap > 0 ? (uint32_t)sw().bits_qcap
                                         : (uint32_t)std::min(512.0, 64.0 + 32.0 * std::ceil(2.0 * per_tile / 32.0));
        while (qc > 64u && fixed + FZ_WAVES_PER_BLOCK * fz_wave_lds_pref_bytes(qc, fa.win_pieces) > budget) qc -= 32u;
        fa.qcap = qc;
        fused_lds = fixed + FZ_WAVES_PER_BLOCK * fz_wave_lds_pref_bytes(fa.qcap, fa.win_pieces);
        if (fused_lds > kFusedLdsBudget) bits_nw = 0;
        else fa.fused = 1u;
    }
    bool adapt_plain = false;
    if (!bits_nw && fa.fused && in_memory && with_verify && !sw().no_bits && per_tile > 16.0 && q.mode == FZ_MODE_SUBS) {
        const uint32_t fixed = mpad + FZ_TABLE_BYTES;
        uint32_t qc = sw().bits_qcap > 0 ? (uint32_t)sw().bits_qcap : (uint32_t)std::min(512.0, 64.0 + 32.0 * std::ceil(2.0 * per_tile / 32.0));
        while (qc > 64u && fixed + FZ_WAVES_PER_BLOCK * fz_wave_lds_pref_bytes(qc, fa.win_pieces) > target + 4096) qc -= 32u;
        if (fixed + FZ_WAVES_PER_BLOCK * fz_wave_lds_pref_bytes(qc, fa.win_pieces) <= kFusedLdsBudget) {
            adapt_plain = true;
            fa.qcap = qc;
            fused_lds = fixed + FZ_WAVES_PER_BLOCK * fz_wave_lds_pref_bytes(qc, fa.win_pieces);
        }
    }
    const bool no_wf_fuse = sw().no_wf_fuse;
    const uint32_t wf_fused_lds = mpad + FZ_TABLE_BYTES + FZ_WAVES_PER_BLOCK * fz_wave_lds_bytes(fz_wf_fused_dwords(fa.win_dwords, (uint32_t)vp.gw), 0, 1, true);
    const int wf32_env = sw().wf32;
    const bool wf_candidate = !bits_nw && !fa.fused && in_memory && with_verify && !force_big && !no_wf_fuse && vp.want_wf && !vp.big && vp.gw <= 32 &&
                              q.m <= FZ_MAX_M && wf_fused_lds <= target + 4096;
    const bool wf_fused = wf_candidate && (vp.gw == 16 || (wf32_env >= 0 ? wf32_env != 0 : per_tile > 0.1));
    if (wf_fused) { fa.fused = 1u; fused_lds = wf_fused_lds; fa.vlanes = 64; }
    sp.wfg = bits_nw ? bits_nw : adapt_plain ? 3 : wf_fused ? vp.gw : 0;
    sp.form = !with_verify ? FZ_FORM_NONE : bits_nw == 4 ? FZ_FORM_FUSED_BITS32 : bits_nw == 1 ? FZ_FORM_FUSED_BITS1 : bits_nw == 2 ? FZ_FORM_FUSED_BITS2
              : wf_fused ? FZ_FORM_FUSED_CELLS : fa.fused ? FZ_FORM_FUSED_BAND : FZ_FORM_KERNEL;
    sp.lds = fa.fused ? fused_lds : FZ_TABLE_BYTES + FZ_WAVES_PER_BLOCK * fz_wave_lds_bytes(0, 0, 64, true);
    sp.overlapped = shares_chip && fa.fused && in_memory && !partial && q.m <= FZ_MAX_M && !vp.big;

    constexpr uint64_t kTilesPerWg = 12;
    const uint64_t resident = (uint64_t)n_cus * 6;
    uint64_t max_grid = std::max<uint64_t>(resident, ntiles / kTilesPerWg);
    if (ntiles < resident * 120) {
        const uint64_t rounds = std::max<uint64_t>(1, (2 * ntiles + resident * 19 / 2) / (resident * 19));
        max_grid = resident * rounds;
    }
    constexpr uint64_t kTilesPerWgOverlapped = 16;
    constexpr bool kTaperOverlapped = false;
    if (sp.overlapped) max_grid = std::max<uint64_t>(resident, ntiles / kTilesPerWgOverlapped);
    const uint64_t min_grid = (ntiles + FZ_TITER_MAX - 1) / FZ_TITER_MAX;
    sp.grid = (uint32_t)std::max<uint64_t>(std::max<uint64_t>(1, min_grid), std::min<uint64_t>(ntiles, max_grid));
    if (!sp.overlapped || kTaperOverlapped) plan_scan_regions(fa, ntiles, sp.grid, n_cus);
    else fa.nreg = 0;
    if (partial) {
        fa.nreg = 1;
        fa.reg_wg0[0] = 0; fa.reg_nwg[0] = sp.grid; fa.reg_tile0[0] = tile_lo; fa.reg_end[0] = tile_hi;
    }
    return sp;
}

uint32_t fill_launch_blocks(FzScanArgs &fa, const Search &q, uint32_t g0, const HashGeom &hgeom) {
    const uint32_t L = q.plan.L, G = (uint32_t)q.plan.s.size();
    uint32_t hash_k = 0, lut_shift = 0;
    const uint32_t nblk = choose_launch_blocks(q.p, q.plan.s.data(), g0, G, L, hash_k, lut_shift);
    fa.hash_k = hash_k;
    fa.lut_shift = lut_shift;
    fa.nblk = nblk;
    fa.g0 = g0;
    for (uint32_t b = 0; b < nblk; ++b) {
        const uint8_t *ng = q.p + q.plan.s[g0 + b];
        fa.A[b] = load_le32(ng, L) & fa.mask1;
        fa.B[b] = hgeom.nwin == 2 ? load_le32(ng + fa.d2, 4) : 0;
        fa.H[b] = hgeom.nwin == 2 ? fz_hash_windows(fa.A[b], load_le32(ng + hgeom.dh, 3), fa.hash_k) : fz_hash_short(fa.A[b], fa.hash_k);
        fa.s[b] = q.plan.s[g0 + b];
        fz_block_range(q.mode, q.m, q.k, L, fa.s[b], fa.lo_rel[b], fa.hi_sub[b]);
    }
    fa.flags = q.any ? FZ_FLAG_ANY : 0u;
    for (uint32_t b = 1; b < nblk; ++b)
        for (uint32_t c = 0; c < b; ++c)
            if (fa.H[b] == fa.H[c]) fa.flags |= FZ_FLAG_DUP_HASHES;
    return nblk;
}

int enqueue_shard(fz_ctx *ctx, const Shard &sh, const Search &q, bool with_verify, bool copy_back = true, bool behind = false) {
    DevState &d = lane_dev(ctx, sh.dev);
    HIP_TRY(hipSetDevice(d.device));
    unsigned long long *counters = reinterpret_cast<unsigned long long *>(d.d_out);
    FzRec *recs = reinterpret_cast<FzRec *>(d.d_out + kHeaderBytes);
    const bool no_direct = env_no_direct();
    const bool snapshot = copy_back && with_verify && q.collective;
    const bool direct = copy_back && d.direct && !no_direct && !snapshot && sh.geom.buf_len > 0 && !q.plan.s.empty();
    if (direct && with_verify) recs = reinterpret_cast<FzRec *>(d.cur().h_stage_dev + kHeaderBytes);
    SearchRun &run = d.cur().run = SearchRun{};
    run.last_direct = direct;
    run.timed = ctx->timing;

    FzScanArgs fa;
    fill_common_args(fa, sh, q);
    const ScanPlan sp = plan_scan(q, sh.geom, (uint32_t)d.n_cus, with_verify, behind && ctx->streams == 2 && direct, fa);
    const VerifyPlan &vp = sp.vp;
    const uint32_t L = q.plan.L;
    const uint32_t G = (uint32_t)q.plan.s.size();
    const uint64_t ntiles = sp.ntiles;
    const dim3 grid(sp.grid);
    if (q.mode == FZ_MODE_GENERIC && !with_verify) fa.gen_dedup = d.gen_dedup_arg;
    {
        int rc = stage_pattern(d, fa, q.p, q.m, with_verify && vp.big);
        if (rc) return rc;
    }
    const HashGeom hgeom(L);
    const int nwin = hgeom.nwin, dh = hgeom.dh;
    fa.d2 = nwin == 2 ? std::min<uint32_t>(L, 8) - 4 : 0;
    fa.mask1 = hgeom.mask1;
    fa.mask2 = 0xffffffffu;
    fa.hit_cap = d.hit_cap;
    fa.rec_cap = direct ? kHostRecs : d.rec_cap;
    if (sp.overlapped && fa.pat_g) return fail(FZ_EDEVICE, "internal: an overlapped scan with the pattern staged in HBM");
    const bool alt = sp.overlapped && !d.slots[d.slot_id ^ 1].run.on_alt;
    run.on_alt = alt;
    const hipStream_t st = alt ? d.stream_alt : d.stream;
    if (alt) counters = reinterpret_cast<unsigned long long *>(d.d_hdr_alt);
    else {
        if (!d.header_zeroed) HIP_TRY(hipMemsetAsync(d.d_out, 0, kHeaderBytes, d.stream));
        d.header_zeroed = false;
    }

    const bool ext_events = copy_back && direct && !(with_verify && !fa.fused) && ntiles > 0 && G > 0;
    const bool attach = ntiles > 0 && G > 0;
    if (ctx->timing && !attach) HIP_TRY(hipEventRecord(d.cur().ev[0], st));
    uint32_t launches = 0;
    for (uint32_t g0 = 0; g0 < G && ntiles > 0;) {
        const uint32_t nblk = fill_launch_blocks(fa, q, g0, hgeom);
        const bool verify_follows = with_verify && !fa.fused;
        fa.host_hdr = (direct && !verify_follows && g0 + nblk >= G) ? reinterpret_cast<uint64_t>(d.cur().h_stage_dev) : 0;
        const bool ragged = geom_is_ragged(sh.geom);
        const bool seg = sh.geom.seg_stride != 0;
        ScanKernel kern = ragged ? batch_scan_kernel(nwin, dh, fa.fused != 0, fa.lut_shift == 2, sp.wfg)
                          : scan_is_lean(q.mode, q.k, fa, sp.wfg, seg, ragged) ? lean_scan_kernel(nwin, dh, fa.lut_shift == 2)
                          : scan_kernel(nwin, dh, fa.fused != 0, seg, fa.lut_shift == 2, sp.wfg);
        if (!kern) return fail(FZ_EUNSUPPORTED, "this (lab) build carries no scan kernel for nwin=%d dh=%d", nwin, dh);
        hipEvent_t ev_start = (attach && ctx->timing && g0 == 0) ? d.cur().ev[0] : nullptr;
        hipEvent_t ev_stop = g0 + nblk >= G ? (ext_events ? d.cur().ev[3] : (attach && ctx->timing) ? d.cur().ev[1] : nullptr) : nullptr;
        launch(kern, grid, dim3(FZ_FILTER_THREADS), sp.lds, st, ev_start, ev_stop, sh.d_buf, fa, ntiles, d.d_hits, recs, counters);
        HIP_TRY(hipGetLastError());
        ++launches;
        g0 += nblk;
    }
    run.scan_end_event = (copy_back && direct && !(with_verify && !fa.fused)) ? 3 : 1;
    if (run.scan_end_event == 1 && ctx->timing && !attach) HIP_TRY(hipEventRecord(d.cur().ev[1], st));
    hipEvent_t v_stop = (copy_back && direct && !snapshot) ? d.cur().ev[3] : nullptr;
    if (with_verify && !fa.fused && ntiles > 0 && G > 0) {
        run.verify_launched = true;
        if (v_stop) run.verify_end_event = 3;
        fa.nblk = 0;
        fa.g0 = 0;
        fa.host_hdr = direct ? reinterpret_cast<uint64_t>(d.cur().h_stage_dev) : 0;
        using VerifyKernel = void (*)(const uint8_t *, const FzScanArgs, const uint64_t *, FzRec *, unsigned long long *);
        VerifyKernel vk;
        dim3 vgrid, vblock;
        size_t vlds;
        if (vp.big) {
            if (!fa.pat_g) return fail(FZ_EDEVICE, "internal: the pattern was not staged for the big verification");
            const uint32_t cells = q.mode == FZ_MODE_LEV ? 2 * q.k + 1 : 1;
            const bool rag = geom_is_ragged(sh.geom);
            if (cells <= 64) vk = rag ? fz_batch_verify_big_kernel<1> : fz_verify_big_kernel<1>;
            else if (cells <= 128) vk = rag ? fz_batch_verify_big_kernel<2> : fz_verify_big_kernel<2>;
            else if (cells <= 256) vk = rag ? fz_batch_verify_big_kernel<4> : fz_verify_big_kernel<4>;
            else if (cells <= 512) vk = rag ? fz_batch_verify_big_kernel<16> : fz_verify_big_kernel<8>;
            else if (cells <= 1024) vk = rag ? fz_batch_verify_big_kernel<16> : fz_verify_big_kernel<16>;
            else vk = rag ? fz_batch_verify_big_kernel<32> : fz_verify_big_kernel<32>;
            vgrid = dim3(d.n_cus * 32); vblock = dim3(64); vlds = 0;
        } else if (vp.want_wf) {
            fa.gw = (uint32_t)vp.gw;
            const bool rag = geom_is_ragged(sh.geom);
            if (vp.gw == 16) vk = rag ? fz_batch_verify_wf_kernel<16> : fz_verify_wf_kernel<16>;
            else if (vp.gw == 32) vk = rag ? fz_batch_verify_wf_kernel<32> : fz_verify_wf_kernel<32>;
            else vk = rag ? fz_batch_verify_wf_kernel<64> : fz_verify_wf_kernel<64>;
            vgrid = dim3(d.n_cus * 2); vblock = dim3(1024); vlds = vp.wf_lds;
        } else {
            fa.vlanes = 64;
            vk = geom_is_ragged(sh.geom) ? fz_batch_verify_kernel : fz_verify_kernel;
            if (vp.ring_lds > 64 * 1024)
                HIP_TRY(hipFuncSetAttribute(reinterpret_cast<const void *>(vk), hipFuncAttributeMaxDynamicSharedMemorySize, (int)vp.ring_lds));
            vgrid = dim3(d.n_cus * 4); vblock = dim3(64 * vp.waves); vlds = vp.ring_lds;
        }
        launch(vk, vgrid, vblock, (uint32_t)vlds, d.stream, nullptr, v_stop, sh.d_buf, fa, d.d_hits, recs, counters);
        HIP_TRY(hipGetLastError());
    }
    const bool completion_attached = ext_events || (run.verify_launched && v_stop);
    if (copy_back) {
        if (run.verify_launched && ctx->timing && run.verify_end_event == 2) HIP_TRY(hipEventRecord(d.cur().ev[2], d.stream));
        if (snapshot) {
            HIP_TRY(hipMemcpyAsync(d.cur().h_stage, d.d_out, kHeaderBytes, hipMemcpyDeviceToHost, d.stream));
            int rc = ensure_send(d, d.rec_cap);
            if (rc) return rc;
            HIP_TRY(hipMemcpyAsync(d.cur().d_send, d.d_out, kHeaderBytes + d.rec_cap * sizeof(FzRec), hipMemcpyDeviceToDevice, d.stream));
            HIP_TRY(hipEventRecord(d.cur().ev_snap, d.stream));
            d.cur().snap_taken = true;
        } else if (!direct) {
            d.first_copy = std::min<uint64_t>(std::min<uint64_t>(d.first_copy, kFirstCopyRecs), d.rec_cap);
            HIP_TRY(hipMemcpyAsync(d.cur().h_stage, d.d_out, kHeaderBytes + d.first_copy * sizeof(FzRec), hipMemcpyDeviceToHost,
                                   d.stream));
        }
        if (!completion_attached) HIP_TRY(hipEventRecord(d.cur().ev[3], st));
        if (!direct) HIP_TRY(hipMemsetAsync(d.d_out, 0, kHeaderBytes, d.stream));
        if (!alt) d.header_zeroed = true;
    }
    run.launches_used = launches;
    run.fused_used = fa.fused != 0;
    run.form_used = sp.form;
    run.hit_cap_used = d.hit_cap;
    run.rec_cap_used = d.rec_cap;
    return FZ_OK;
}

// ... 180 lines not shown
#define NCCL_TRY(expr)                                                                             \
    do {                                                                                           \
        ncclResult_t r_ = (expr);                                                                  \
        if (r_ != ncclSuccess) return fail(FZ_EDEVICE, "%s failed: %s", #expr, rccl_api()->GetErrorString(r_)); \
    } while (0)

int comm_wait(hipStream_t st, const char *what) {
    const auto t0 = std::chrono::steady_clock::now();
    const long limit_ms = sw().comm_timeout_ms;
    for (;;) {
        const hipError_t e = hipStreamQuery(st);
        if (e == hipSuccess) return FZ_OK;
        (void)hipGetLastError();
        if (e != hipErrorNotReady) return fail(FZ_EDEVICE, "%s: %s", what, hipGetErrorString(e));
        const auto waited = std::chrono::steady_clock::now() - t0;
        if (waited > std::chrono::milliseconds(limit_ms))
            return fail(FZ_ETIMEOUT, "%s did not complete within %ld ms (FZ_COMM_TIMEOUT_MS): a rank of the communicator never arrived",
                        what, limit_ms);
        if (waited > std::chrono::microseconds(200)) std::this_thread::sleep_for(std::chrono::microseconds(20));
    }
}

int gather_records(fz_ctx *ctx, fz_seq *seq, std::vector<FzRec> &recs) {
    const int world = ctx->comm_world;
    if (world <= 0) return fail(FZ_EINVAL, "the context has not joined a communicator");
    if (ctx->comm_broken) return fail(FZ_ETIMEOUT, "the communicator was abandoned after a collective ran into its deadline: "
                                                   "fz_comm_set_collective(ctx, 0) searches without it");
    recs.clear();
    const auto t_start = std::chrono::steady_clock::now();
    int rcl = comm_rank_lows(ctx, seq);
    if (rcl) return rcl;
    for (int attempt = 0; attempt < 8; ++attempt) {
        const uint64_t bytes = kHeaderBytes + ctx->gcap * sizeof(FzRec);
        for (DevState &d : ctx->devs) {
            HIP_TRY(hipSetDevice(d.device));
            int rc = ensure_send(d, std::max<uint64_t>(d.rec_cap, ctx->gcap));
            if (rc) return rc;
            if (d.recv_bytes < (uint64_t)world * bytes) {
                HIP_TRY(hipStreamSynchronize(d.comm_stream));
                if (d.d_recv) HIP_TRY(hipFree(d.d_recv));
                if (d.h_recv) HIP_TRY(hipHostFree(d.h_recv));
                d.d_recv = nullptr; d.h_recv = nullptr; d.recv_bytes = 0;
                HIP_TRY(hipMalloc(reinterpret_cast<void **>(&d.d_recv), (uint64_t)world * bytes));
                HIP_TRY(hipHostMalloc(reinterpret_cast<void **>(&d.h_recv), (uint64_t)world * bytes, hipHostMallocDefault));
                d.recv_bytes = (uint64_t)world * bytes;
            }
            bool has_shard = false;
            for (const Shard &sh : seq->shards) has_shard |= &ctx->devs[sh.dev] == &d;
            if (has_shard && d.cur().snap_taken) HIP_TRY(hipStreamWaitEvent(d.comm_stream, d.cur().ev_snap, 0));
            else HIP_TRY(hipMemsetAsync(d.cur().d_send, 0, kHeaderBytes, d.comm_stream));
        }
        NCCL_TRY(rccl_api()->GroupStart());
        for (DevState &d : ctx->devs)
            NCCL_TRY(rccl_api()->AllGather(d.cur().d_send, d.d_recv, bytes, ncclChar, d.comm, d.comm_stream));
        NCCL_TRY(rccl_api()->GroupEnd());
        DevState &d0 = ctx->devs[0];
        HIP_TRY(hipSetDevice(d0.device));
        HIP_TRY(hipMemcpyAsync(d0.h_recv, d0.d_recv, (uint64_t)world * bytes, hipMemcpyDeviceToHost, d0.comm_stream));
        HIP_TRY(hipEventRecord(d0.ev_done, d0.comm_stream));
        {
            int rcw = comm_wait(d0.comm_stream, "the all-gather of the ranks' records");
            if (rcw) { if (rcw == FZ_ETIMEOUT) ctx->comm_broken = true; return rcw; }
        }
        for (size_t i = 1; i < ctx->devs.size(); ++i) {
            HIP_TRY(hipSetDevice(ctx->devs[i].device));
            int rcw = comm_wait(ctx->devs[i].comm_stream, "the all-gather of the ranks' records");
            if (rcw) { if (rcw == FZ_ETIMEOUT) ctx->comm_broken = true; return rcw; }
        }
        uint64_t top = 0, total = 0;
        parse_gathered(d0.h_recv, world, bytes, ctx->gcap, seq->rank_lo.data(), recs, ctx->seg_ends, ctx->seg_order, &top, &total);
        if (top > ctx->gcap) {
            ctx->gcap = (top + top / 4 + 1023) / 1024 * 1024;
            continue;
        }
        ctx->stats.raw_matches = total;
        const uint64_t want = std::max<uint64_t>(1024, (top + top / 4 + 1023) / 1024 * 1024);
        if (want * 2 <= ctx->gcap) ctx->gcap = want;
        ctx->last_gather_ms = std::chrono::duration<double, std::milli>(std::chrono::steady_clock::now() - t_start).count();
        return FZ_OK;
    }
    return fail(FZ_EDEVICE, "all-gather capacity kept overflowing");
}

int search_enqueue(fz_ctx *ctx, fz_seq *seq, const Search &q, bool with_verify, bool behind = false) {
    ctx->view = nullptr;
    ctx->view_n = 0;
    ctx->rows_ready = false;
    ctx->stats.filter_launches = 0;
    ctx->stats.bytes_scanned = ctx->stats.ngram_hits = ctx->stats.raw_matches = 0;
    ctx->stats.filter_ms = ctx->stats.verify_ms = ctx->stats.device_ms = 0;
    ctx->tref.clear();
    int rc = for_each_shard(ctx, seq, [ctx, seq, &q, with_verify, behind](size_t si) {
        return enqueue_shard(ctx, seq->shards[si], q, with_verify, true, behind);
    });
    if (rc) return rc;
    for (const Shard &sh : seq->shards) {
        const SearchRun &run = lane_dev(ctx, sh.dev).cur().run;
        ctx->stats.filter_launches += run.launches_used;
        ctx->stats.verify_form = run.form_used;
    }
    return FZ_OK;
}

int emit_matches(const FzRec *recs, size_t cnt, uint32_t L, fz_match **out, uint64_t *n, uint64_t idx_bound, uint32_t blk_bound,
                 bool may_have_empty, std::vector<fz_match> *into);

int search_collect(fz_ctx *ctx, fz_seq *seq, const Search &q, bool with_verify, std::vector<FzRec> &recs,
                   std::vector<uint64_t> &hits) {
    const size_t ns = seq->shards.size();
    if (ctx->souts.size() < ns) ctx->souts.resize(ns);
    const bool order_rows = with_verify && !q.collective && ns > 1 && !q.any && seq->shards[0].geom.seg_stride == 0;
    for (int attempt = 0; attempt < 4; ++attempt) {
        recs.clear();
        hits.clear();
        ctx->rows_ready = false;
        ctx->stats.bytes_scanned = ctx->stats.ngram_hits = ctx->stats.raw_matches = 0;
        ctx->stats.filter_ms = ctx->stats.verify_ms = ctx->stats.device_ms = 0;
        ctx->tref.clear();
        Trace tr;
        ctx->seg_ends.clear();
        ctx->seg_order.clear();
        const uint32_t L = q.plan.L, nblk = (uint32_t)q.plan.s.size();
        const uint64_t nglob = seq->n;
        const bool collective = q.collective;
        int rc = for_each_shard(ctx, seq, [ctx, seq, with_verify, ns, collective, order_rows, L, nblk, nglob](size_t si) {
            ShardOut &so = ctx->souts[si];
            int r = collect_shard(ctx, seq->shards[si], with_verify, ns == 1, so, collective);
            if (r || so.rerun || !order_rows) return r;
            const bool dense = ctx->devs[seq->shards[si].dev].cur().run.fused_used;
            return emit_matches(so.recs.data(), so.recs.size(), L, nullptr, nullptr, nglob, nblk, !dense, &so.rows);
        });
        if (rc) return rc;
        bool any_rerun = false;
        for (size_t si = 0; si < ns; ++si) {
            ShardOut &so = ctx->souts[si];
            any_rerun |= so.rerun;
            if (so.rerun) continue;
            ctx->stats.bytes_scanned += so.bytes;
            ctx->stats.ngram_hits += so.nh;
            ctx->stats.raw_matches += so.nr;
            if (so.tref.d) ctx->tref.push_back(so.tref);
        }
        tr.mark(" collect");
        if (!any_rerun) {
            if (with_verify && q.collective) {
                int rc2 = gather_records(ctx, seq, recs);
                if (rc2) return rc2;
                tr.mark(" all-gather");
                return FZ_OK;
            }
            if (ns == 1) {
                recs.swap(ctx->souts[0].recs);
                hits.swap(ctx->souts[0].hits);
            } else if (order_rows) {
                ctx->rows_ready = true;
                for (uint32_t si = 0; si < ns; ++si) ctx->seg_order.push_back(si);
                std::sort(ctx->seg_order.begin(), ctx->seg_order.end(), [&](uint32_t x, uint32_t y) {
                    return seq->shards[x].geom.own_lo < seq->shards[y].geom.own_lo;
                });
            } else {
                for (size_t si = 0; si < ns; ++si) {
                    recs.insert(recs.end(), ctx->souts[si].recs.begin(), ctx->souts[si].recs.end());
                    hits.insert(hits.end(), ctx->souts[si].hits.begin(), ctx->souts[si].hits.end());
                }
            }
            return FZ_OK;
        }
        rc = search_enqueue(ctx, seq, q, with_verify);
        if (rc) return rc;
    }
    return fail(FZ_EDEVICE, "result buffers kept overflowing");
}

int run_search(fz_ctx *ctx, fz_seq *seq, const Search &q, bool with_verify, std::vector<FzRec> &recs,
               std::vector<uint64_t> &hits) {
    if (ctx->npend) return fail(FZ_EINVAL, "a search started with fz_lev_ngrams_begin is still in flight");
    memset(&ctx->stats, 0, sizeof ctx->stats); ctx->tref.clear();
    ctx->stats.n_devices = (uint32_t)ctx->devs.size();
    Trace tr;
    int rc = search_enqueue(ctx, seq, q, with_verify);
    if (rc) return rc;
    tr.mark(" enqueue");
    return search_collect(ctx, seq, q, with_verify, recs, hits);
}

using GhKernel = void (*)(const uint8_t *, const FzScanArgs, const uint64_t *, FzGenRec *, unsigned long long *);
struct GenHitPlan {
    GhKernel kernel;
    bool bits;
    uint32_t waves;
    uint32_t capw;
    size_t lds;
};

GenHitPlan plan_gen_hit(const Search &q, uint32_t cand_cap) {
    GenHitPlan g;
    const uint32_t mpad = (q.m + 15u) & ~15u, wpad = (q.m + 2 * q.k + 15u) & ~15u;
    static_assert(FZ_MAX_K < (1u << 31), "fz_b_lt / fz_b_eq operands");
    g.bits = q.m <= 64u && q.k <= 32u && q.m >= 1u && q.m + 2u * q.k <= 128u &&
             std::max(std::max(q.max_subs, q.max_ins), std::max(q.max_dels, q.k)) <= FZ_MAX_K && !sw().gh_no_bits;
    const uint32_t env = (uint32_t)sw().gh_waves;
    g.waves = env == 4u || env == 2u || (env == 1u && g.bits) ? env : g.bits ? 1u : 2u;
    g.capw = g.waves == 1u ? std::max<uint32_t>(64u, cand_cap) : std::max<uint32_t>(64u, cand_cap / 2u);
    g.lds = (size_t)mpad + wpad + FZ_GH_CTL_BYTES + (size_t)g.waves * 2u * g.capw * sizeof(FzGCand) +
            (size_t)g.waves * FZ_GH_MCAP_W(g.waves) * 8u +
            (g.bits ? (size_t)FZ_GH_PT_BYTES + (size_t)wpad * 8u + (size_t)64u * g.waves * 8u : 0u);
    g.kernel = g.bits ? (g.waves == 1u ? fz_gen_hit_kernel<1, true> : g.waves == 2u ? fz_gen_hit_kernel<2, true> : fz_gen_hit_kernel<4, true>)
                      : (g.waves == 4u ? fz_gen_hit_kernel<4, false> : fz_gen_hit_kernel<2, false>);
    return g;
}

int run_generic(fz_ctx *ctx, fz_seq *seq, const Search &q, std::vector<FzGenRec> &recs_out, int phase = 0) {
    memset(&ctx->stats, 0, sizeof ctx->stats); ctx->tref.clear();
    ctx->stats.n_devices = (uint32_t)ctx->devs.size();
    static_assert(sizeof(FzGenRec) == sizeof(FzRec), "record buffers are shared");
    uint32_t cand_cap = ctx->gen_cand_cap;
    bool legacy_rest = false;
    for (int attempt = 0; attempt < 10; ++attempt) {
        recs_out.clear();
        ctx->any_found = false;
        ctx->gen_view = nullptr;
        ctx->gen_view_n = 0;
        ctx->gen_rows_dev = nullptr;
        ctx->gen_rows_n = 0;
        bool rerun = false;
        bool multi_failed = false, multi_ok = false;
        const bool legacy_now = legacy_rest || (attempt == 0 && phase != 2 && ctx->gen_multi_skip > 0);
        if (attempt == 0 && phase != 2 && ctx->gen_multi_skip > 0) { --ctx->gen_multi_skip; legacy_rest = true; }
        ctx->stats.filter_launches = 0;
        ctx->stats.bytes_scanned = ctx->stats.ngram_hits = ctx->stats.raw_matches = 0;
        ctx->stats.filter_ms = ctx->stats.verify_ms = ctx->stats.device_ms = 0;
        ctx->tref.clear();
        const uint32_t mpad = (q.m + 15u) & ~15u, wpad = (q.m + 2 * q.k + 15u) & ~15u;
        for (const Shard &sh : seq->shards) {
            if (phase == 2 && attempt == 0) break;
            DevState &d = lane_dev(ctx, sh.dev);
            const bool dev_order = !q.any && !q.fold && seq->shards.size() == 1 && sh.geom.seg_stride == 0 && !comm_multi_process(ctx);
            const bool dedup = !sw().gen_no_dedup && sh.geom.seg_stride == 0 && (dev_order || q.fold || q.any);
            d.gen_dedup_arg = 0;
            if (dedup) {
                HIP_TRY(hipSetDevice(d.device));
                if (!d.d_gen_dedup) {
                    HIP_TRY(hipMalloc(reinterpret_cast<void **>(&d.d_gen_dedup), FZ_GEN_DEDUP_BYTES));
                    d.dedup_zeroed = false;
                }
                if (!d.dedup_zeroed) HIP_TRY(hipMemsetAsync(d.d_gen_dedup, 0, FZ_GEN_DEDUP_ZERO_BYTES, d.stream));
                d.dedup_zeroed = false;
                d.gen_dedup_arg = reinterpret_cast<uint64_t>(d.d_gen_dedup);
            }
            int rc = enqueue_shard(ctx, sh, q, false, false);
            if (rc) return rc;
            SearchRun &run = d.cur().run;
            run.dedup_used = dedup;
            size_t lds = 0;
            uint64_t scratch = 0;
            rc = cand_lists(d, cand_cap, mpad + wpad + FZ_GEN_MCAP * 8, lds, scratch);
            if (rc) return rc;
            FzScanArgs fa;
            fill_common_args(fa, sh, q);
            rc = stage_pattern(d, fa, q.p, q.m);
            if (rc) return rc;
            fa.flags = (q.any ? FZ_FLAG_ANY : 0u) | (q.fold ? FZ_FLAG_FOLD : 0u);
            fa.cand_cap = cand_cap;
            fa.cand_scratch = scratch;
            fa.lp_kind = FZ_LP_GENERIC_HIT;
            fa.lp_starts = 0;
            rc = ensure_big(d, 1u << 16);
            if (rc) return rc;
            fa.hit_cap = d.hit_cap;
            if (dev_order) {
                rc = ensure_gen_rows(d);
                if (rc) return rc;
                fa.gen_order = reinterpret_cast<uint64_t>(d.d_gen_order);
                fa.rows_cap = d.gen_rows_cap;
            }
            fa.gen_dedup = d.gen_dedup_arg;
            const bool fold_direct = q.fold && !env_no_direct() && d.fold_direct && seq->shards.size() == 1;
            run.fold_was_direct = fold_direct;
            fa.rec_cap = fold_direct ? kHostRecs : d.rec_cap;
            if (fold_direct) fa.host_hdr = reinterpret_cast<uint64_t>(d.cur().h_stage_dev);
            unsigned long long *counters = reinterpret_cast<unsigned long long *>(d.d_out);
            FzGenRec *recs = reinterpret_cast<FzGenRec *>((fold_direct ? d.cur().h_stage_dev : d.d_out) + kHeaderBytes);
            static_assert(sizeof(FzGenRec) == sizeof(FzRec), "the generic records share the record buffer");
            const GenHitPlan gp = plan_gen_hit(q, cand_cap);
            const bool multi = ctx->gen_multi && !legacy_now && scratch == 0 && sh.geom.seg_stride == 0 && gp.lds <= 160 * 1024;
            run.gen_multi_used = multi;
            if (multi) {
                fa.cand_cap = gp.capw;
                if (gp.lds > 64 * 1024)
                    HIP_TRY(hipFuncSetAttribute(reinterpret_cast<const void *>(gp.kernel), hipFuncAttributeMaxDynamicSharedMemorySize, (int)gp.lds));
            }
            const LpKernel lp = lp_kernel(FZ_LP_GENERIC_HIT, scratch != 0);
            if (lds > 64 * 1024)
                HIP_TRY(hipFuncSetAttribute(reinterpret_cast<const void *>(lp), hipFuncAttributeMaxDynamicSharedMemorySize, (int)lds));
            constexpr unsigned kLpGridPerCu = 24;
            constexpr unsigned kGenHitGridPerCu = 32;
            hipEvent_t lp_stop = fold_direct ? d.cur().ev[3] : ctx->timing ? d.cur().ev[2] : nullptr;
            run.lp_end_event = fold_direct ? 3 : 2;
            if (multi)
                launch(gp.kernel, dim3(d.n_cus * kGenHitGridPerCu), dim3(64 * gp.waves), (uint32_t)gp.lds, d.stream, nullptr, lp_stop,
                       sh.d_buf, fa, d.d_hits, recs, counters);
            else
                launch(lp, dim3(scratch ? kCandScratchGrid : d.n_cus * kLpGridPerCu), dim3(64), (uint32_t)lds, d.stream, nullptr, lp_stop,
                       sh.d_buf, fa, d.d_hits, (uint64_t)0, recs, counters);
            HIP_TRY(hipGetLastError());
            if (ctx->timing && !lp_stop && !fold_direct) HIP_TRY(hipEventRecord(d.cur().ev[2], d.stream));
            if (dev_order) {
                hipLaunchKernelGGL(fz_gen_order_kernel, dim3(d.n_cus * 8), dim3(256), 0, d.stream, d.d_hits, fa, counters);
                hipLaunchKernelGGL(fz_gen_scatter_kernel, dim3(d.n_cus * 8), dim3(256), 0, d.stream, d.d_hits, fa, recs,
                                   reinterpret_cast<FzOutRow *>(d.d_gen_rows), counters);
                HIP_TRY(hipGetLastError());
            }
            run.fold_copied = fold_direct ? kHostRecs : q.fold ? std::min<uint64_t>(std::min<uint64_t>(d.fold_guess, kHostRecs), d.rec_cap) : 0;
            if (!fold_direct) {
                HIP_TRY(hipMemcpyAsync(d.cur().h_stage, d.d_out, kHeaderBytes + run.fold_copied * sizeof(FzGenRec), hipMemcpyDeviceToHost, d.stream));
                HIP_TRY(hipEventRecord(d.cur().ev[3], d.stream));
                HIP_TRY(hipMemsetAsync(d.d_out, 0, kHeaderBytes, d.stream));
            } else {
                if (!lp_stop) HIP_TRY(hipEventRecord(d.cur().ev[3], d.stream));
            }
            d.header_zeroed = true;
            if (dedup) {
                HIP_TRY(hipMemsetAsync(d.d_gen_dedup, 0, FZ_GEN_DEDUP_ZERO_BYTES, d.stream));
                d.dedup_zeroed = true;
            }
        }
        if (phase == 1) return FZ_OK;
        bool lists_overflowed = false;
        Trace trg;
        trg.mark(" generic enqueue");
        for (const Shard &sh : seq->shards) {
            DevState &d = lane_dev(ctx, sh.dev);
            const SearchRun &run = d.cur().run;
// ... 3534 lines not shown
    if (ctx->devs.size() != 1) return fail(FZ_EINVAL, "fz_comm_allgather is for one-process-per-GPU jobs (a multi-device context holds every rank's data itself)");
    if (!nbytes) return FZ_OK;
    if (!send || !recv) return fail(FZ_EINVAL, "null argument");
    return comm_allgather_fixed(ctx, send, nbytes, recv);
}

int fz_comm_max_f64(fz_ctx *ctx, double *value) {
    int rc = comm_busy(ctx);
    if (rc) return rc;
    if (!ctx->comm_world || !value) return fail(FZ_EINVAL, "no communicator / null argument");
    if (ctx->devs.size() != 1) return FZ_OK;
    if (ctx->comm_broken) return fail(FZ_ETIMEOUT, "the communicator was abandoned after a collective ran into its deadline");
    DevState &d = ctx->devs[0];
    HIP_TRY(hipSetDevice(d.device));
    double *tmp = nullptr;
    HIP_TRY(hipMalloc(reinterpret_cast<void **>(&tmp), sizeof(double)));
    auto body = [&]() -> int {
        HIP_TRY(hipMemcpyAsync(tmp, value, sizeof(double), hipMemcpyHostToDevice, d.comm_stream));
        NCCL_TRY(rccl_api()->AllReduce(tmp, tmp, 1, ncclDouble, ncclMax, d.comm, d.comm_stream));
        HIP_TRY(hipMemcpyAsync(value, tmp, sizeof(double), hipMemcpyDeviceToHost, d.comm_stream));
        return comm_wait(d.comm_stream, "an all-reduce over the job's ranks");
    };
    rc = body();
    if (rc == FZ_ETIMEOUT) ctx->comm_broken = true;
    else (void)hipFree(tmp);
    return rc;
}

int fz_comm_barrier(fz_ctx *ctx) {
    if (ctx) for (DevState &d : ctx->devs) { (void)hipSetDevice(d.device); (void)hipStreamSynchronize(d.stream); (void)hipStreamSynchronize(d.stream_alt); }
    double one = 1.0;
    return fz_comm_max_f64(ctx, &one);
}

void fz_debug_reload_switches(void) { switches_storage() = read_switches(); }

int fz_comm_backend(void) { return !rccl_api()->ok ? 0 : rccl_api()->stand_in ? 2 : 1; }

int fz_comm_gather_ms(fz_ctx *ctx, double *ms) {
    if (!ctx || !ms) return fail(FZ_EINVAL, "null argument");
    *ms = ctx->last_gather_ms;
    return FZ_OK;
}

int fz_debug_scan_regions(uint64_t ntiles, uint64_t grid, uint32_t n_cus, int steps, double fmin, int wg_per_cu, uint32_t *n_regions,
                          uint64_t *table) {
    if (!n_regions || !table) return fail(FZ_EINVAL, "null argument");
    static FzScanArgs fa;
    static std::mutex mu;
    std::lock_guard<std::mutex> lk(mu);
    plan_scan_regions(fa, ntiles, grid, n_cus, steps, fmin, wg_per_cu);
    *n_regions = fa.nreg;
    for (uint32_t r = 0; r < fa.nreg; ++r) {
        table[4 * r] = fa.reg_wg0[r]; table[4 * r + 1] = fa.reg_nwg[r]; table[4 * r + 2] = fa.reg_tile0[r]; table[4 * r + 3] = fa.reg_end[r];
    }
    return FZ_OK;
}

int fz_debug_scan_plan(const uint8_t *p, uint32_t m, uint32_t k, uint64_t buf_len, uint32_t n_cus, int shares_chip, uint32_t *grid,
                       uint32_t *form, int *overlapped, uint32_t *n_regions, uint64_t *table) {
    if (!p || !grid || !form || !overlapped || !n_regions || !table || m == 0 || m / (k + 1) == 0 || n_cus == 0)
        return fail(FZ_EINVAL, "bad argument");
    Search q;
    q.mode = FZ_MODE_LEV; q.m = m; q.k = k; q.p = p;
    q.plan.L = m / (k + 1);
    for (uint32_t s = 0; s + q.plan.L <= m; s += q.plan.L) q.plan.s.push_back(s);
    FzGeom geom{};
    geom.buf_len = buf_len;
    static FzScanArgs fa;
    static std::mutex mu;
    std::lock_guard<std::mutex> lk(mu);
    memset(&fa, 0, sizeof fa);
    const ScanPlan sp = plan_scan(q, geom, n_cus, true, shares_chip != 0, fa);
    *grid = sp.grid;
    *form = sp.form;
    *overlapped = sp.overlapped ? 1 : 0;
    *n_regions = fa.nreg;
    for (uint32_t r = 0; r < fa.nreg; ++r) {
        table[4 * r] = fa.reg_wg0[r]; table[4 * r + 1] = fa.reg_nwg[r]; table[4 * r + 2] = fa.reg_tile0[r]; table[4 * r + 3] = fa.reg_end[r];
    }
    return FZ_OK;
}

int fz_debug_scan_instance(uint32_t mode, const uint8_t *p, uint32_t m, uint32_t k, uint64_t buf_len, uint32_t n_cus,
                           uint32_t *n_launches, uint32_t *lean_mask, uint32_t *form) {
    if (!p || !n_launches || !lean_mask || !form || m == 0 || m / (k + 1) == 0 || n_cus == 0 || (mode != FZ_MODE_LEV && mode != FZ_MODE_SUBS))
        return fail(FZ_EINVAL, "bad argument");
    Search q;
    q.mode = mode; q.m = m; q.k = k; q.p = p;
    q.plan.L = m / (k + 1);
    for (uint32_t s = 0; s + q.plan.L <= m; s += q.plan.L) q.plan.s.push_back(s);
    if (q.plan.s.size() > FZ_MAX_BLOCKS) return fail(FZ_EUNSUPPORTED, "more than %u n-gram blocks", FZ_MAX_BLOCKS);
    FzGeom geom{};
    geom.buf_len = buf_len;
    static FzScanArgs fa;
    static std::mutex mu;
    std::lock_guard<std::mutex> lk(mu);
    memset(&fa, 0, sizeof fa);
    const ScanPlan sp = plan_scan(q, geom, n_cus, true, false, fa);
    const HashGeom hgeom(q.plan.L);
    fa.d2 = hgeom.nwin == 2 ? std::min<uint32_t>(q.plan.L, 8) - 4 : 0;
    fa.mask1 = hgeom.mask1;
    uint32_t nl = 0, mask = 0;
    for (uint32_t g0 = 0; g0 < q.plan.s.size(); ++nl) {
        const uint32_t nblk = fill_launch_blocks(fa, q, g0, hgeom);
        if (nblk == 0) return fail(FZ_EDEVICE, "internal: a launch without blocks");
        if (nl < 32 && scan_is_lean(q.mode, q.k, fa, sp.wfg, false, false)) mask |= 1u << nl;
        g0 += nblk;
    }
    *n_launches = nl;
    *lean_mask = mask;
    *form = sp.form;
    return FZ_OK;
}

int fz_debug_gather_merge(const void *blocks, uint32_t world, uint64_t cap, const uint64_t *own_lo, uint32_t L, fz_match **out,
                          uint64_t *n_out, uint64_t *need_cap) {
    if (!blocks || !out || !n_out || !need_cap || world == 0) return fail(FZ_EINVAL, "null argument");
    *out = nullptr; *n_out = 0; *need_cap = 0;
    std::vector<FzRec> recs;
    std::vector<size_t> seg_ends;
    std::vector<uint32_t> seg_order;
    uint64_t top = 0, total = 0;
    parse_gathered(static_cast<const uint8_t *>(blocks), (int)world, kHeaderBytes + cap * sizeof(FzRec), cap, own_lo, recs, seg_ends,
                   seg_order, &top, &total);
    if (top > cap) { *need_cap = (top + top / 4 + 1023) / 1024 * 1024; return FZ_OK; }
    return emit_matches_segments(nullptr, recs.data(), seg_ends, seg_order, L, out, n_out, 0, 0, true);
}

}

namespace {

struct LpRec { int64_t start, end; int32_t dist; uint64_t step; uint64_t w0; uint32_t seq; };

constexpr uint32_t kLpStarts = 256;

int run_lp(fz_ctx *ctx, fz_seq *seq, const Search &q, uint32_t lp_kind, std::vector<LpRec> &out) {
    if ((uint64_t)q.m + 2ull * q.k + kLpStarts > 65535ull)
        return fail(FZ_EUNSUPPORTED, "linear-programming route: len(subsequence) + 2 * max_l_dist + %u = %llu exceeds 65535 (16-bit window coordinates)",
                    kLpStarts, (unsigned long long)q.m + 2ull * q.k + kLpStarts);
    memset(&ctx->stats, 0, sizeof ctx->stats); ctx->tref.clear();
    ctx->stats.n_devices = (uint32_t)ctx->devs.size();
    uint32_t cand_cap = 1024;
    for (int attempt = 0; attempt < 8; ++attempt) {
        out.clear();
        bool rerun = false;
        const uint32_t mpad = (q.m + 15u) & ~15u, wpad = (q.m + 2 * q.k + kLpStarts + 15u) & ~15u;
        for (const Shard &sh : seq->shards) {
            DevState &d = ctx->devs[sh.dev];
            HIP_TRY(hipSetDevice(d.device));
            size_t lds = 0;
            uint64_t scratch = 0;
            int rc_lists = cand_lists(d, cand_cap, mpad + wpad + FZ_GEN_MCAP * 8, lds, scratch);
            if (rc_lists) return rc_lists;
            unsigned long long *counters = reinterpret_cast<unsigned long long *>(d.d_out);
            FzGenRec *recs = reinterpret_cast<FzGenRec *>(d.d_out + kHeaderBytes);
            HIP_TRY(hipMemsetAsync(d.d_out, 0, kHeaderBytes, d.stream));
            d.header_zeroed = false;
            HIP_TRY(hipEventRecord(d.cur().ev[0], d.stream));
            FzScanArgs fa;
            memset(&fa, 0, sizeof fa);
            fa.geom = sh.geom;
            fa.mode = q.mode; fa.m = q.m; fa.k = q.k; fa.L = 0;
            fa.max_subs = q.max_subs; fa.max_ins = q.max_ins; fa.max_dels = q.max_dels;
            fa.cand_cap = cand_cap;
// ... 292 lines not shown
    if (st->mode == FZ_MODE_GENERIC) {
        std::vector<FzGenRec> recs;
        rc = run_generic(ctx, st->seq, st->q, recs);
        if (rc) return rc;
        rc = emit_generic(ctx, st->seq, recs, L, st->k, &mo, &cnt, &so);
        if (rc) return rc;
    } else {
        std::vector<FzRec> recs;
        std::vector<uint64_t> hits;
        const bool with_verify = st->mode != FZ_MODE_EXACT;
        rc = search_collect(ctx, st->seq, st->q, with_verify, recs, hits);
        if (rc) return rc;
        if (st->mode == FZ_MODE_LEV) {
            const FzRec *r = ctx->view ? ctx->view : recs.data();
            const size_t nr = ctx->view ? (size_t)ctx->view_n : recs.size();
            rc = emit_matches_seg(r, nr, L, &mo, &cnt, &so);
            if (rc) return rc;
        } else {
            std::vector<fz_match> tmp;
            if (st->mode == FZ_MODE_EXACT) {
                std::sort(hits.begin(), hits.end());
                tmp.resize(hits.size());
                for (size_t i = 0; i < hits.size(); ++i) {
                    const int64_t idx = (int64_t)fz_hit_index(hits[i]);
                    tmp[i] = fz_match{idx, idx + (int64_t)st->m, 0, 0};
                }
            } else {
                fz_match *em = nullptr;
                uint64_t en = 0;
                rc = emit_matches(ctx, recs, L, &em, &en);
                if (rc) return rc;
                tmp.assign(em, em + en);
                release_out(em);
            }
            std::vector<std::pair<uint64_t, uint32_t>> order;
            for (size_t i = 0; i < tmp.size(); ++i) {
                const uint64_t j = stream_window_segment(st, (uint64_t)tmp[i].start);
                if (j >= st->fl_j0 && j < st->fl_j1) order.emplace_back(j, (uint32_t)i);
            }
            std::stable_sort(order.begin(), order.end(), [](const std::pair<uint64_t, uint32_t> &x, const std::pair<uint64_t, uint32_t> &y) { return x.first < y.first; });
            for (const auto &o : order) { st->out.push_back(tmp[o.second]); st->out_seg.push_back((uint32_t)o.first); }
            return FZ_OK;
        }
    }
    st->out.insert(st->out.end(), mo, mo + cnt);
    st->out_seg.insert(st->out_seg.end(), so, so + cnt);
    release_out(mo);
    release_out(so);
    return FZ_OK;
}

int stream_launch(fz_stream *st, uint64_t j0, uint64_t j1, uint64_t data_hi) {
    fz_ctx *ctx = st->ctx;
    if (ctx->npend || (ctx->stream_inflight && ctx->stream_inflight != st))
        return fail(FZ_EINVAL, "another search or file stream of this context is in flight");
    DevState &d = ctx->devs[0];
    Shard &sh = st->seq->shards[0];
    HIP_TRY(hipSetDevice(d.device));
    const uint64_t len = data_hi - st->stage_off;
    FzGeom g{};
    g.n = data_hi;
    g.buf_off = st->stage_off;
    g.buf_len = len;
    g.own_lo = 0;
    g.own_hi = data_hi;
    const bool segmented = st->mode == FZ_MODE_LEV || st->mode == FZ_MODE_GENERIC;
    if (segmented) {
        g.seg_stride = st->S; g.seg_org = 0; g.seg_pre = st->pre; g.seg_post = st->post;
        g.seg_j0 = j0; g.seg_j1 = j1;
    }
    sh.geom = g;
    st->seq->n = data_hi;
    if (len) HIP_TRY(hipMemcpyAsync(sh.d_buf, st->h_buf[st->cur], len, hipMemcpyHostToDevice, d.stream));
    const uint64_t tiles = (len + FZ_TILE_BYTES - 1) / FZ_TILE_BYTES;
    const uint64_t body = std::max<uint64_t>(1, tiles) * FZ_TILE_BYTES;
    HIP_TRY(hipMemsetAsync(sh.d_buf + len, 0, body + FZ_PAD_BACK - len, d.stream));
    st->fl_j0 = j0;
    st->fl_j1 = j1;
    int rc = ensure_hits(d, std::max<uint64_t>(1u << 20, len / 64));
    if (rc) return rc;
    if (st->mode != FZ_MODE_GENERIC) {
        memset(&ctx->stats, 0, sizeof ctx->stats); ctx->tref.clear();
        ctx->stats.n_devices = 1;
        rc = search_enqueue(ctx, st->seq, st->q, st->mode != FZ_MODE_EXACT);
        if (rc) return rc;
    }
    st->inflight = true;
    ctx->stream_inflight = st;
    return FZ_OK;
}

}

extern "C" {

int fz_stream_open(fz_ctx *ctx, uint32_t mode, const uint8_t *p, uint32_t m, uint32_t max_subs, uint32_t max_ins,
                   uint32_t max_dels, uint32_t k, uint64_t seg_stride, uint32_t seg_pre, uint32_t seg_post,
                   uint64_t batch_bytes, fz_stream **out) {
    if (!out) return fail(FZ_EINVAL, "null argument");
    *out = nullptr;
    if (!ctx || ctx->devs.empty()) return fail(FZ_EINVAL, "bad ctx handle");
    if (ctx->devs.size() != 1) return fail(FZ_EUNSUPPORTED, "file streams run on a single-device context");
    if (ctx->npend || ctx->stream_inflight) return fail(FZ_EINVAL, "another search of this context is in flight");
    if (!p || m == 0) return fail(FZ_EINVAL, "subsequence must not be empty");
    if (m > FZ_MAX_M_ANY) return fail(FZ_EUNSUPPORTED, "subsequence longer than %u bytes", FZ_MAX_M_ANY);
    if (mode > FZ_MODE_GENERIC) return fail(FZ_EINVAL, "bad mode");
    if (mode == FZ_MODE_GENERIC && (uint64_t)m + 2ull * k > 65535ull)
        return fail(FZ_EUNSUPPORTED, "generic search: len(subsequence) + 2 * max_l_dist exceeds 65535 (16-bit window coordinates)");
    if (k > (mode == FZ_MODE_GENERIC ? (uint32_t)FZ_MAX_K : FZ_MAX_K_ANY)) return fail(FZ_EUNSUPPORTED, "distance limit %u is not supported", k);
    if (seg_stride == 0 || (seg_pre && seg_post)) return fail(FZ_EINVAL, "bad segment geometry");
    if ((uint64_t)seg_pre + seg_post > seg_stride / 2 || (uint64_t)m + 2ull * k + 2 > seg_stride)
        return fail(FZ_EUNSUPPORTED, "chunk too small for this pattern (use the per-chunk path)");
    fz_stream *st = new (std::nothrow) fz_stream();
    if (!st) return fail(FZ_ENOMEM, "out of memory");
    st->ctx = ctx;
    st->mode = mode; st->m = m; st->k = k;
    st->max_subs = std::min(max_subs, 255u); st->max_ins = std::min(max_ins, 255u); st->max_dels = std::min(max_dels, 255u);
    st->pat.assign(p, p + m);
    st->S = seg_stride; st->pre = seg_pre; st->post = seg_post;
    int rc = stream_build_search(st);
    if (rc) { delete st; return rc; }
    const uint64_t ext = (uint64_t)seg_pre + seg_post;
    st->cap = std::max<uint64_t>(batch_bytes, seg_stride + ext) + seg_stride + ext;
    DevState &d = ctx->devs[0];
    auto init = [&]() -> int {
        HIP_TRY(hipSetDevice(d.device));
        const uint64_t need_d = FZ_PAD_FRONT + ((st->cap + FZ_TILE_BYTES - 1) / FZ_TILE_BYTES + 1) * FZ_TILE_BYTES + FZ_PAD_BACK;
        uint8_t *cached_d = nullptr;
        if (d.stream_h[0] && d.stream_cap >= st->cap && d.stream_d_bytes >= need_d) {
            st->h_buf[0] = d.stream_h[0]; st->h_buf[1] = d.stream_h[1];
            cached_d = d.stream_d;
            st->cap_alloc = d.stream_cap;
            d.stream_h[0] = d.stream_h[1] = nullptr; d.stream_d = nullptr;
        } else {
            for (int i = 0; i < 2; ++i) HIP_TRY(hipHostMalloc(reinterpret_cast<void **>(&st->h_buf[i]), st->cap, hipHostMallocDefault));
            st->cap_alloc = st->cap;
        }
        st->seq = new (std::nothrow) fz_seq();
        if (!st->seq) return fail(FZ_ENOMEM, "out of memory");
        st->seq->ctx = ctx;
        st->seq->shards.emplace_back();
        Shard &sh = st->seq->shards[0];
        sh.dev = 0;
        if (cached_d) {
            sh.d_alloc = cached_d;
            sh.alloc_bytes = d.stream_d_bytes;
        } else {
            sh.alloc_bytes = need_d;
            HIP_TRY(hipMalloc(reinterpret_cast<void **>(&sh.d_alloc), sh.alloc_bytes));
        }
        sh.d_buf = sh.d_alloc + FZ_PAD_FRONT;
        HIP_TRY(hipMemsetAsync(sh.d_alloc, 0, FZ_PAD_FRONT, d.stream));
        return FZ_OK;
    };
    rc = init();
    if (rc) { fz_stream_close(st); return rc; }
    *out = st;
    return FZ_OK;
}

int fz_stream_buffer(fz_stream *st, uint8_t **host, uint64_t *capacity) {
    if (!st || !host || !capacity) return fail(FZ_EINVAL, "null argument");
    *host = st->h_buf[st->cur] + st->stage_len;
    *capacity = st->eof ? 0 : st->cap - st->stage_len;
    return FZ_OK;
}

// ... 602 lines not shown
    for (uint64_t i = 0; i < n; ++i) {
        if (!slot[i]) continue;
        const uint32_t c = slot[i] - 1;
        fz_match best = in[members[first[c]]];
        for (uint32_t q = first[c] + 1; q < first[c + 1]; ++q)
            if (better(in[members[q]], best)) best = in[members[q]];
        o[w++] = best;
    }
    *out = o;
    *n_out = w;
    return FZ_OK;
}

static int group_best_exact(const fz_match *in, uint64_t n, fz_match **out, uint64_t *n_out) {
    struct Key {
        int64_t s, e; uint64_t seq;
        bool operator<(const Key &o) const { return s != o.s ? s < o.s : (e != o.e ? e < o.e : seq < o.seq); }
    };
    auto better = [](const fz_match &a, const fz_match &b) {
        const int64_t la = a.end - a.start, lb = b.end - b.start;
        return a.dist < b.dist || (a.dist == b.dist && (la > lb || (la == lb && a.start < b.start)));
    };
    std::map<Key, fz_match> groups;
    uint64_t next_seq = 0;
    std::vector<std::map<Key, fz_match>::iterator> ov;
    for (uint64_t i = 0; i < n; ++i) {
        const fz_match &mt = in[i];
        auto overlaps = [&](const Key &g) { return !(mt.end <= g.s || mt.start >= g.e); };
        ov.clear();
        auto it = groups.lower_bound(Key{mt.start, INT64_MIN, 0});
        for (auto pb = it; pb != groups.begin();) {
            --pb;
            if (pb->first.e == pb->first.s) continue;
            if (overlaps(pb->first)) ov.push_back(pb);
            break;
        }
        for (; it != groups.end() && it->first.s < mt.end; ++it)
            if (overlaps(it->first)) ov.push_back(it);
        if (ov.empty()) {
            groups.emplace(Key{mt.start, mt.end, next_seq++}, mt);
        } else if (ov.size() == 1 && mt.start >= ov[0]->first.s && mt.end <= ov[0]->first.e) {
            if (better(mt, ov[0]->second)) ov[0]->second = mt;
        } else if (ov.size() == 1) {
            auto node = groups.extract(ov[0]);
            node.key().s = std::min(node.key().s, mt.start);
            node.key().e = std::max(node.key().e, mt.end);
            if (better(mt, node.mapped())) node.mapped() = mt;
            groups.insert(std::move(node));
        } else {
            std::sort(ov.begin(), ov.end(), [](const auto &x, const auto &y) { return x->first.seq < y->first.seq; });
            Key u{mt.start, mt.end, 0};
            fz_match best = mt;
            for (auto g : ov) {
                u.s = std::min(u.s, g->first.s);
                u.e = std::max(u.e, g->first.e);
                if (better(g->second, best)) best = g->second;
            }
            for (auto g : ov) groups.erase(g);
            u.seq = next_seq++;
            groups.emplace(u, best);
        }
    }
    std::vector<std::pair<uint64_t, fz_match>> ordered;
    ordered.reserve(groups.size());
    for (const auto &g : groups) ordered.emplace_back(g.first.seq, g.second);
    std::sort(ordered.begin(), ordered.end(), [](const auto &x, const auto &y) { return x.first < y.first; });
    void *mem = nullptr;
    int rc = alloc_out(ordered.size(), sizeof(fz_match), &mem);
    if (rc) return rc;
    fz_match *o = static_cast<fz_match *>(mem);
    for (size_t g = 0; g < ordered.size(); ++g) o[g] = ordered[g].second;
    *out = o;
    *n_out = ordered.size();
    return FZ_OK;
}

int fz_set_timing(fz_ctx *ctx, int on) {
    if (!ctx) return fail(FZ_EINVAL, "null argument");
    if (ctx->npend || ctx->stream_inflight) return fail(FZ_EINVAL, "a search of this context is in flight");
    ctx->timing = on != 0;
    return FZ_OK;
}

int fz_set_streams(fz_ctx *ctx, int n) {
    if (!ctx || (n != 1 && n != 2)) return fail(FZ_EINVAL, "streams must be 1 or 2");
    if (ctx->npend || ctx->stream_inflight) return fail(FZ_EINVAL, "a search of this context is in flight");
    ctx->streams = n;
    return FZ_OK;
}

int fz_stats(fz_ctx *ctx, fz_stats_t *out) {
    if (!ctx || !out) return fail(FZ_EINVAL, "null argument");
    resolve_timing(ctx);
    *out = ctx->stats;
    return FZ_OK;
}

int fz_mem_info(fz_ctx *ctx, uint64_t *free_bytes, uint64_t *total_bytes) {
    if (!ctx || !free_bytes || !total_bytes) return fail(FZ_EINVAL, "null argument");
    uint64_t fmin = ~0ull, tmin = ~0ull;
    for (const DevState &d : ctx->devs) {
        HIP_TRY(hipSetDevice(d.device));
        size_t f = 0, t = 0;
        HIP_TRY(hipMemGetInfo(&f, &t));
        fmin = std::min<uint64_t>(fmin, f);
        tmin = std::min<uint64_t>(tmin, t);
    }
    *free_bytes = fmin;
    *total_bytes = tmin;
    return FZ_OK;
}

void fz_free(void *p) { release_out(p); }


}
```

include/fzhip.h:

```cpp
#ifndef FZHIP_H
#define FZHIP_H

#include <stdint.h>

#ifdef __cplusplus
extern "C" {
#endif

#define FZ_ABI_VERSION 1

#define FZ_OK          0
#define FZ_EINVAL     -1
#define FZ_ENOMEM     -2
#define FZ_EDEVICE    -3
#define FZ_EUNSUPPORTED -4
#define FZ_EHALO      -5
#define FZ_ETIMEOUT   -6

typedef struct fz_ctx fz_ctx;
typedef struct fz_seq fz_seq;

typedef struct {
    int64_t start, end;
    int32_t dist;
// ... 185 lines not shown
int fz_debug_derive_ms(fz_ctx *ctx, double *ms5);

int fz_batch_upload_records_lines(fz_ctx *ctx, const uint8_t *text, uint64_t n, uint32_t lines_per_record, const uint32_t *lines,
                                  uint32_t n_kept, uint32_t flags, fz_seq **outs, fz_records_info *info);

#define FZ_FORMAT_MAX_COLUMNS 8u
#define FZ_FORMAT_MAX_LITERAL 255u
#define FZ_FORMAT_NO_CHECK 0xffffffffu
typedef struct {
    uint64_t n_records, text_bytes, longest_record, bad_record;
    uint32_t bad_reason;
} fz_format_info;

int fz_batch_format(fz_ctx *ctx, fz_seq *const *columns, uint32_t n_columns, const uint8_t *literals, const uint32_t *literal_lens,
                    uint32_t equal_a, uint32_t equal_b, uint8_t *out, uint64_t cap, fz_format_info *info);
int fz_debug_format_plan(const uint64_t *const *offs, uint32_t n_columns, uint64_t n, const uint32_t *literal_lens,
                         uint32_t equal_a, uint32_t equal_b, uint64_t *at, fz_format_info *info);
int fz_debug_format_ms(fz_ctx *ctx, double *ms5);

int fz_subs_ngrams_any(fz_ctx *ctx, fz_seq *seq, const uint8_t *p, uint32_t m, uint32_t k, int *found);
int fz_subs_lp_any(fz_ctx *ctx, fz_seq *seq, const uint8_t *p, uint32_t m, uint32_t k, int *found);
int fz_generic_ngrams_any(fz_ctx *ctx, fz_seq *seq, const uint8_t *p, uint32_t m,
                          uint32_t max_subs, uint32_t max_ins, uint32_t max_dels, uint32_t max_l, int *found);

int fz_lev_lp(fz_ctx *ctx, fz_seq *seq, const uint8_t *p, uint32_t m, uint32_t k, fz_match **out, uint64_t *n);
int fz_subs_lp(fz_ctx *ctx, fz_seq *seq, const uint8_t *p, uint32_t m, uint32_t k, fz_match **out, uint64_t *n);
int fz_generic_lp(fz_ctx *ctx, fz_seq *seq, const uint8_t *p, uint32_t m,
                  uint32_t max_subs, uint32_t max_ins, uint32_t max_dels, uint32_t max_l,
                  fz_match **out, uint64_t *n);

#define FZ_COMM_ID_BYTES 128
int  fz_comm_unique_id(void *id, uint64_t id_bytes);
int  fz_comm_init_rank(fz_ctx *ctx, const void *id, int world, int rank);
int  fz_comm_init_all(fz_ctx *ctx);
int  fz_comm_info(fz_ctx *ctx, int *world, int *rank, int *collective);
int  fz_comm_set_collective(fz_ctx *ctx, int on);
int  fz_comm_allgather(fz_ctx *ctx, const void *send, uint64_t nbytes, void *recv);
int  fz_comm_max_f64(fz_ctx *ctx, double *value);
int  fz_comm_barrier(fz_ctx *ctx);
void fz_comm_destroy(fz_ctx *ctx);
int  fz_comm_gather_ms(fz_ctx *ctx, double *ms);
int  fz_comm_backend(void);

int fz_consolidate(const fz_match *in, uint64_t n, fz_match **out, uint64_t *n_out);

int fz_group_best(const fz_match *in, uint64_t n, fz_match **out, uint64_t *n_out);

int fz_merge_ranks(const fz_match *const *parts, const uint64_t *counts, const uint64_t *block_counts,
                   uint32_t world, uint32_t nb, fz_match *out);

#define FZ_WIRE_HEADER_ROWS 65
int fz_wire_pack(const fz_match *in, uint64_t n, uint64_t cap_rows, void *dst);
int fz_wire_merge(const void *recv, uint32_t world, uint64_t rows_per_rank, uint64_t cap_rows,
                  fz_match *out, uint64_t out_cap, uint64_t *n_out, uint64_t *max_count);

typedef struct fz_stream fz_stream;
int  fz_stream_open(fz_ctx *ctx, uint32_t mode, const uint8_t *p, uint32_t m, uint32_t max_subs, uint32_t max_ins,
                    uint32_t max_dels, uint32_t k, uint64_t seg_stride, uint32_t seg_pre, uint32_t seg_post,
                    uint64_t batch_bytes, fz_stream **out);
int  fz_stream_buffer(fz_stream *st, uint8_t **host, uint64_t *capacity);
int  fz_stream_submit(fz_stream *st, uint64_t nbytes, int last);
int  fz_stream_read_fd(fz_stream *st, int fd, int64_t offset, int threads, uint64_t *total);
int  fz_stream_finish(fz_stream *st, fz_match **out, uint32_t **seg, uint64_t *n);
void fz_stream_close(fz_stream *st);

void fz_debug_reload_switches(void);

int fz_debug_launch_plan(const uint8_t *p, uint32_t m, uint32_t L, uint32_t *out, uint32_t cap, uint32_t *n_launches);

int fz_debug_order_records(const void *recs, uint64_t n, uint32_t L, fz_match **out, uint64_t *n_out);
int fz_debug_order_records_bounded(const void *recs, uint64_t n, uint32_t L, uint64_t idx_bound, uint32_t blk_bound,
                                   fz_match **out, uint64_t *n_out);
int fz_debug_order_segments(const void *recs, const uint64_t *seg_ends, uint32_t n_segments, uint32_t L, fz_match **out, uint64_t *n_out);

int fz_debug_scan_regions(uint64_t ntiles, uint64_t grid, uint32_t n_cus, int steps, double fmin, int wg_per_cu, uint32_t *n_regions,
                          uint64_t *table);

int fz_debug_scan_plan(const uint8_t *p, uint32_t m, uint32_t k, uint64_t buf_len, uint32_t n_cus, int shares_chip, uint32_t *grid,
                       uint32_t *form, int *overlapped, uint32_t *n_regions, uint64_t *table);

int fz_debug_scan_instance(uint32_t mode, const uint8_t *p, uint32_t m, uint32_t k, uint64_t buf_len, uint32_t n_cus,
                           uint32_t *n_launches, uint32_t *lean_mask, uint32_t *form);

int fz_debug_gather_merge(const void *blocks, uint32_t world, uint64_t cap, const uint64_t *own_lo, uint32_t L, fz_match **out,
                          uint64_t *n_out, uint64_t *need_cap);

int  fz_stats(fz_ctx *ctx, fz_stats_t *out);
int  fz_mem_info(fz_ctx *ctx, uint64_t *free_bytes, uint64_t *total_bytes);
int  fz_set_timing(fz_ctx *ctx, int on);
int  fz_set_streams(fz_ctx *ctx, int n);
int  fz_device_ms(fz_ctx *ctx, double *filter_ms, int cap);
void fz_free(void *p);

#ifdef __cplusplus
}
#endif
#endif
```

Before: 5490.

## Alternate scan direction between launches to reuse cache-resident tail of the buffer

```diff
diff --git a/fuzzysearch_amd/_native.py b/fuzzysearch_amd/_native.py
--- a/fuzzysearch_amd/_native.py
+++ b/fuzzysearch_amd/_native.py
@@ -166,11 +166,14 @@
     "fz_debug_scan_regions": (ci, (u64, u64, u32, ci, f64, ci, u32p, vp)),
     "fz_debug_scan_plan": (ci, (cs, u32, u32, u64, u32, ci, u32p, u32p, cip, u32p, vp)),
     "fz_debug_scan_instance": (ci, (u32, cs, u32, u32, u64, u32, u32p, u32p, u32p)),
+    "fz_debug_scan_walk": (ci, (u64, u32, u32, vp, u32, u32, ci, u64p)),
+    "fz_debug_scan_direction": (ci, (vp, vp, cip, u64p)),
     "fz_debug_gather_merge": (ci, (vp, u32, u64, vp, u32, mpp, u64p, u64p)),
     "fz_stats": (ci, (vp, stp)),
     "fz_mem_info": (ci, (vp, u64p, u64p)),
     "fz_set_timing": (ci, (vp, ci)),
     "fz_set_streams": (ci, (vp, ci)),
+    "fz_set_scan_direction": (ci, (vp, ci)),
     "fz_device_ms": (ci, (vp, f64p, ci)),
     "fz_free": (None, (vp,)),
 }
@@ -188,6 +191,7 @@
     "fz_batch_derive", "fz_debug_derive_plan", "fz_debug_derive_ms",
     "fz_batch_upload_records_lines", "fz_batch_format", "fz_debug_format_plan", "fz_debug_format_ms",
     "fz_debug_scan_plan", "fz_mem_info", "fz_debug_scan_instance",
+    "fz_debug_scan_walk", "fz_debug_scan_direction", "fz_set_scan_direction",
 ))
 
 _lib = None
@@ -1274,6 +1278,17 @@
         with self._lock:
             _check(self._lib.fz_set_streams(self._h, n))
 
+    def set_scan_direction(self, mode):
+        with self._lock:
+            _check(_entry(self._lib, "fz_set_scan_direction")(self._h, mode))
+
+    def scan_direction(self, seq=None):
+        nxt, cnt = ci(0), u64(0)
+        with self._lock:
+            _check(_entry(self._lib, "fz_debug_scan_direction")(self._h, seq._h if seq is not None else None,
+                                                                 ctypes.byref(nxt), ctypes.byref(cnt)))
+        return bool(nxt.value), cnt.value
+
     def stats(self):
         st = FzStats()
         with self._lock:
diff --git a/fuzzysearch_amd/csrc/fz_device.h b/fuzzysearch_amd/csrc/fz_device.h
--- a/fuzzysearch_amd/csrc/fz_device.h
+++ b/fuzzysearch_amd/csrc/fz_device.h
@@ -171,6 +171,33 @@
     uint32_t reg_wg0[FZ_MAX_REGIONS], reg_nwg[FZ_MAX_REGIONS];
     uint64_t reg_tile0[FZ_MAX_REGIONS], reg_end[FZ_MAX_REGIONS];
 };
+
+struct FzWalk {
+    uint64_t first, limit;
+    uint32_t stride;
+    uint64_t phys_first;
+    int32_t phys_stride;
+};
+FZ_HD uint64_t fz_walk_phys(uint64_t ntiles, uint64_t logical, bool rev) { return rev ? ntiles - 1u - logical : logical; }
+FZ_HD FzWalk fz_scan_walk(uint32_t nreg, const uint32_t *reg_wg0, const uint32_t *reg_nwg, const uint64_t *reg_tile0,
+                          const uint64_t *reg_end, uint32_t grid, uint64_t ntiles, uint32_t wg, bool rev) {
+    uint32_t wg0 = 0, stride = grid;
+    uint64_t tile0 = 0, limit = ntiles;
+#pragma unroll
+    for (uint32_t r = 0; r < FZ_MAX_REGIONS; ++r)
+        if (r < nreg && wg >= reg_wg0[r]) { wg0 = reg_wg0[r]; stride = reg_nwg[r]; tile0 = reg_tile0[r]; limit = reg_end[r]; }
+    FzWalk w;
+    w.first = tile0 + (wg - wg0);
+    w.limit = limit;
+    w.stride = stride;
+    w.phys_first = fz_walk_phys(ntiles, w.first, rev);
+    w.phys_stride = rev ? -(int32_t)stride : (int32_t)stride;
+    return w;
+}
+FZ_HD uint64_t fz_walk_tile(const FzWalk &w, uint32_t iter) {
+    if (w.first + (uint64_t)iter * w.stride >= w.limit) return ~0ull;
+    return (uint64_t)((int64_t)w.phys_first + (int64_t)iter * (int64_t)w.phys_stride);
+}
 
 #define FZ_IDX_BITS 48
 #define FZ_MAX_BLOCKS 65535u
diff --git a/fuzzysearch_amd/csrc/fz_kernel_bodies.inc b/fuzzysearch_amd/csrc/fz_kernel_bodies.inc
--- a/fuzzysearch_amd/csrc/fz_kernel_bodies.inc
+++ b/fuzzysearch_amd/csrc/fz_kernel_bodies.inc
@@ -40,15 +40,12 @@
     }
     bool dup_hashes = false;
     if constexpr (DUPH) dup_hashes = (a.flags & FZ_FLAG_DUP_HASHES) != 0;
-    uint32_t wg0 = 0, stride = gridDim.x;
-    uint64_t tile0 = 0, limit = ntiles;
-#pragma unroll
-    for (uint32_t r = 0; r < FZ_MAX_REGIONS; ++r)
-        if (r < a.nreg && blockIdx.x >= a.reg_wg0[r]) { wg0 = a.reg_wg0[r]; stride = a.reg_nwg[r]; tile0 = a.reg_tile0[r]; limit = a.reg_end[r]; }
-    const uint64_t first_tile = tile0 + (blockIdx.x - wg0);
+    const FzWalk wk = fz_scan_walk(a.nreg, a.reg_wg0, a.reg_nwg, a.reg_tile0, a.reg_end, gridDim.x, ntiles, blockIdx.x,
+                                   !RAG && !SEG && (a.flags & FZ_FLAG_REVERSE) != 0);
+    const int32_t stride = (int32_t)wk.stride, pstride = wk.phys_stride;
     if (threadIdx.x == 0) {
         uint32_t *walk = reinterpret_cast<uint32_t *>(smem + FZ_WALK_LDS);
-        walk[0] = (uint32_t)first_tile; walk[1] = (uint32_t)(first_tile >> 32); walk[2] = stride;
+        walk[0] = (uint32_t)wk.phys_first; walk[1] = (uint32_t)wk.phys_stride;
     }
     __syncthreads();
     const uint32_t wave = (uint32_t)__builtin_amdgcn_readfirstlane((int)(threadIdx.x >> 6));
@@ -67,8 +64,9 @@
     uint32_t qf = 0;
     uint32_t confirmed = 0;
     uint32_t titer = 0;
-    uint64_t tile = first_tile;
-    if ((a.flags & FZ_FLAG_ANY) && __hip_atomic_load(&counters[1], __ATOMIC_RELAXED, __HIP_MEMORY_SCOPE_AGENT) != 0ull) tile = limit;
+    int32_t left = (int32_t)(wk.limit - wk.first);
+    uint32_t ptile = (uint32_t)wk.phys_first;
+    if ((a.flags & FZ_FLAG_ANY) && __hip_atomic_load(&counters[1], __ATOMIC_RELAXED, __HIP_MEMORY_SCOPE_AGENT) != 0ull) left = 0;
     bool slow = false;
     uint32_t slow_pos = 0;
     uint32_t ylast = 0;
@@ -154,14 +152,14 @@
             if (slow_pos >= steps) {
                 slow = false;
                 if (ADAPT && b0 + bw < a.nblk) b0 += bw;
-                else { b0 = 0; tile += stride; ++titer; }
-            }
-        } else if (tile < limit && (ADAPT ? (qn == 0u || qn + ylast + (ylast >> 2) + 8u <= qcap) : qn <= qcap / 2)) {
+                else { b0 = 0; left -= stride; ptile += (uint32_t)pstride; ++titer; }
+            }
+        } else if (left > 0 && (ADAPT ? (qn == 0u || qn + ylast + (ylast >> 2) + 8u <= qcap) : qn <= qcap / 2)) {
             uint4 va[2], vb[2];
             uint2 ha[2], hb[2];
             bool pre;
             {
-                const uint8_t *tsrc = buf + fz_bcast64(tile * (uint64_t)FZ_TILE_BYTES);
+                const uint8_t *tsrc = buf + fz_bcast64((uint64_t)ptile * FZ_TILE_BYTES);
 #pragma unroll
                 for (int r = 0; r < 2; ++r) {
                     va[r] = *reinterpret_cast<const uint4 *>(tsrc + r * FZ_ROW_BYTES + lane_off);
@@ -169,7 +167,7 @@
                 }
             }
             do {
-                const uint8_t *tsrc = buf + fz_bcast64(tile * (uint64_t)FZ_TILE_BYTES);
+                const uint8_t *tsrc = buf + fz_bcast64((uint64_t)ptile * FZ_TILE_BYTES);
 #pragma unroll
                 for (int r = 0; r < 2; ++r) {
                     vb[r] = *reinterpret_cast<const uint4 *>(tsrc + (r + 2) * FZ_ROW_BYTES + lane_off);
@@ -180,11 +178,12 @@
                 test_row(va[0], ha[0], std::integral_constant<int, 0>{});
                 test_row(va[1], ha[1], std::integral_constant<int, 1>{});
                 const bool same_tile = ADAPT && b0 + bw < a.nblk;
-                const uint64_t next = same_tile ? tile : tile + stride;
-                if constexpr (ADAPT) pre = next < limit && qn + 3u * (qn - q_tile) + 8u <= qcap;
-                else pre = next < limit && qn <= qcap / 2;
+                const int32_t lnext = same_tile ? left : left - stride;
+                const uint32_t pnext = fz_uniform(same_tile ? ptile : ptile + (uint32_t)pstride);
+                if constexpr (ADAPT) pre = lnext > 0 && qn + 3u * (qn - q_tile) + 8u <= qcap;
+                else pre = lnext > 0 && qn <= qcap / 2;
                 {
-                    const uint8_t *nsrc = buf + fz_bcast64((pre ? next : tile) * (uint64_t)FZ_TILE_BYTES);
+                    const uint8_t *nsrc = buf + fz_bcast64((uint64_t)(pre ? pnext : ptile) * FZ_TILE_BYTES);
 #pragma unroll
                     for (int r = 0; r < 2; ++r) {
                         va[r] = *reinterpret_cast<const uint4 *>(nsrc + r * FZ_ROW_BYTES + lane_off);
@@ -214,7 +213,7 @@
                 }
                 if constexpr (ADAPT) ylast = qn - q_tile;
                 if (PREF && qn > qf) {
-                    if (tile) fz_prefetch_tile(buf, a, w, qf, qn, tile * (uint64_t)FZ_TILE_BYTES);
+                    if (ptile) fz_prefetch_tile(buf, a, w, qf, qn, (uint64_t)ptile * FZ_TILE_BYTES);
                     else fz_prefetch_windows(buf, a, w, qf, qn);
                     qf = qn;
                 }
@@ -224,16 +223,18 @@
                     } else {
                         b0 = 0;
                         if (bw < a.nblk && ylast <= (qcap >> 3)) bw <<= 1;
-                        tile = next;
+                        left = lnext;
+                        ptile = pnext;
                         ++titer;
                     }
                 } else {
-                    tile = next;
+                    left = lnext;
+                    ptile = pnext;
                     ++titer;
                 }
             } while (pre);
         }
-        const bool done = !slow && tile >= limit;
+        const bool done = !slow && left <= 0;
         if (PREF && done) break;
         if constexpr (WF) {
             confirmed += fz_flush_wf<WF ? WFG : 16, RAG>(buf, a, smem, pat_lds, w, smem + FZ_TABLE_BYTES + mpad,
diff --git a/fuzzysearch_amd/csrc/fz_kernels.h b/fuzzysearch_amd/csrc/fz_kernels.h
--- a/fuzzysearch_amd/csrc/fz_kernels.h
+++ b/fuzzysearch_amd/csrc/fz_kernels.h
@@ -28,6 +28,7 @@
 #define FZ_FLAG_DUP_HASHES 1u
 #define FZ_FLAG_FOLD 4u
 #define FZ_FLAG_ANY 2u
+#define FZ_FLAG_REVERSE 8u
 #if FZ_LUT_BITS == 5
 #define FZ_LUT_ADDR_MASK_STR "0x7c"
 #else
@@ -354,9 +355,8 @@
 __device__ __forceinline__ uint64_t fz_code_local(uint32_t code, uint32_t &blk) {
     blk = (code >> FZ_TILE_BITS) & (FZ_MAX_BLOCKS_PER_LAUNCH - 1u);
     FzLdsU32 *walk = (FzLdsU32 *)(uintptr_t)FZ_WALK_LDS;
-    const uint64_t first = ((uint64_t)walk[1] << 32) | walk[0];
-    const uint64_t tile = first + (uint64_t)(code >> (FZ_TILE_BITS + FZ_BLK_BITS)) * walk[2];
-    return tile * (uint64_t)FZ_TILE_BYTES + (code & (FZ_TILE_BYTES - 1u));
+    const uint32_t tile = walk[0] + (code >> (FZ_TILE_BITS + FZ_BLK_BITS)) * walk[1];
+    return (uint64_t)tile * FZ_TILE_BYTES + (code & (FZ_TILE_BYTES - 1u));
 }
 
 __device__ __forceinline__ void fz_prefetch_windows(const uint8_t *__restrict__ buf, const FzScanArgs &a,
diff --git a/fuzzysearch_amd/csrc/fzhip.hip b/fuzzysearch_amd/csrc/fzhip.hip
--- a/fuzzysearch_amd/csrc/fzhip.hip
+++ b/fuzzysearch_amd/csrc/fzhip.hip
@@ -46,6 +46,8 @@
     int taper_steps = 4;
     double taper_min = 0.25;
     int taper_wg_per_cu = 7;
+    int scan_dir = 0;
+    bool scan_rounds = false;
     bool no_rccl = false;
     std::string rccl_lib;
     std::string rocm_path = "/opt/rocm";
@@ -70,6 +72,8 @@
         if (const char *e = getenv("ROCM_PATH")) v.rocm_path = e;
         if (const char *e = getenv("FZ_COMM_TIMEOUT_MS")) v.comm_timeout_ms = std::max(1L, atol(e));
         v.mp_force_pass = flag("FZ_MP_FORCE_PASS");
+        if (const char *e = getenv("FZ_SCAN_DIR")) v.scan_dir = !strcmp(e, "fwd") ? 1 : !strcmp(e, "rev") ? 2 : 0;
+        v.scan_rounds = flag("FZ_SCAN_ROUNDS");
         v.trace = flag("FZ_TRACE"); v.stream_trace = flag("FZ_STREAM_TRACE");
         return v;
 }
@@ -214,6 +218,7 @@
     uint8_t *d_buf = nullptr;
     uint64_t alloc_bytes = 0;
     FzGeom geom{};
+    mutable bool scan_at_end = false;
 };
 
 }
@@ -351,6 +356,8 @@
     bool comm_broken = false;
     uint64_t gcap = 4096;
     int streams = 1;
+    int scan_dir = sw().scan_dir;
+    std::atomic<uint64_t> rev_launches{0};
     double last_gather_ms = 0;
     DevWorkers *workers = nullptr;
     std::vector<ShardOut> souts;
@@ -765,6 +772,25 @@
     plan_scan_regions(fa, ntiles, grid, n_cus, steps, fmin, t_per_cu);
 }
 
+void plan_scan_rounds(FzScanArgs &fa, uint64_t ntiles, uint64_t grid, uint32_t n_cus) {
+    fa.nreg = 0;
+    const uint64_t W = (uint64_t)n_cus * (uint64_t)std::max(1, sw().taper_wg_per_cu);
+    if (grid < 2 * W || ntiles < 4 * grid) return;
+    const uint64_t edge = ntiles * W / grid, mid = grid - 2 * W;
+    uint64_t at = 0, wg = 0;
+    auto add = [&](uint64_t nwg, uint64_t tiles) {
+        if (!nwg) return;
+        fa.reg_wg0[fa.nreg] = (uint32_t)wg; fa.reg_nwg[fa.nreg] = (uint32_t)nwg;
+        fa.reg_tile0[fa.nreg] = at; fa.reg_end[fa.nreg] = at + tiles;
+        ++fa.nreg; wg += nwg; at += tiles;
+    };
+    add(W, mid ? edge : ntiles - edge);
+    add(mid, ntiles - 2 * edge);
+    add(W, edge);
+    for (uint32_t r = 0; r < fa.nreg; ++r)
+        if ((fa.reg_end[r] - fa.reg_tile0[r] + fa.reg_nwg[r] - 1) / fa.reg_nwg[r] >= FZ_TITER_MAX) { fa.nreg = 0; break; }
+}
+
 struct ScanPlan {
     uint64_t ntiles = 0;
     uint32_t grid = 1;
@@ -773,6 +799,7 @@
     uint32_t lds = 0;
     VerifyPlan vp;
     bool overlapped = false;
+    bool partial = false;
 };
 
 ScanPlan plan_scan(const Search &q, const FzGeom &geom, uint32_t n_cus, bool with_verify, bool shares_chip, FzScanArgs &fa) {
@@ -783,7 +810,7 @@
     const uint64_t ntiles_all = (geom.buf_len + FZ_TILE_BYTES - 1) / FZ_TILE_BYTES;
     const uint64_t tile_lo = std::min<uint64_t>(ntiles_all, q.part_lo / FZ_TILE_BYTES);
     const uint64_t tile_hi = q.part_hi == ~0ull ? ntiles_all : std::min<uint64_t>(ntiles_all, (q.part_hi + FZ_TILE_BYTES - 1) / FZ_TILE_BYTES);
-    const bool partial = tile_lo != 0 || tile_hi != ntiles_all;
+    const bool partial = sp.partial = tile_lo != 0 || tile_hi != ntiles_all;
     const uint64_t ntiles = sp.ntiles = tile_hi > tile_lo ? tile_hi - tile_lo : 0;
     const bool force_big = sw().force_big_verify;
     sp.vp = plan_verify(q);
@@ -870,6 +897,7 @@
     const uint64_t min_grid = (ntiles + FZ_TITER_MAX - 1) / FZ_TITER_MAX;
     sp.grid = (uint32_t)std::max<uint64_t>(std::max<uint64_t>(1, min_grid), std::min<uint64_t>(ntiles, max_grid));
     if (!sp.overlapped || kTaperOverlapped) plan_scan_regions(fa, ntiles, sp.grid, n_cus);
+    else if (sw().scan_rounds) plan_scan_rounds(fa, ntiles, sp.grid, n_cus);
     else fa.nreg = 0;
     if (partial) {
         fa.nreg = 1;
@@ -901,7 +929,8 @@
     return nblk;
 }
 
-int enqueue_shard(fz_ctx *ctx, const Shard &sh, const Search &q, bool with_verify, bool copy_back = true, bool behind = false) {
+int enqueue_shard(fz_ctx *ctx, const Shard &sh, const Search &q, bool with_verify, bool copy_back = true, bool behind = false,
+                  bool forward = false) {
     DevState &d = lane_dev(ctx, sh.dev);
     HIP_TRY(hipSetDevice(d.device));
     unsigned long long *counters = reinterpret_cast<unsigned long long *>(d.d_out);
@@ -921,6 +950,7 @@
     const uint32_t L = q.plan.L;
     const uint32_t G = (uint32_t)q.plan.s.size();
     const uint64_t ntiles = sp.ntiles;
+    if ((sh.geom.buf_len + FZ_TILE_BYTES - 1) / FZ_TILE_BYTES >> 31) return fail(FZ_EUNSUPPORTED, "a shard of 2^31 tiles or more");
     const dim3 grid(sp.grid);
     if (q.mode == FZ_MODE_GENERIC && !with_verify) fa.gen_dedup = d.gen_dedup_arg;
     {
@@ -948,8 +978,12 @@
     const bool attach = ntiles > 0 && G > 0;
     if (ctx->timing && !attach) HIP_TRY(hipEventRecord(d.cur().ev[0], st));
     uint32_t launches = 0;
+    const bool may_reverse = sh.geom.seg_stride == 0 && !geom_is_ragged(sh.geom) && !sp.partial && !q.any && !forward;
     for (uint32_t g0 = 0; g0 < G && ntiles > 0;) {
         const uint32_t nblk = fill_launch_blocks(fa, q, g0, hgeom);
+        const bool reverse = may_reverse && (ctx->scan_dir == 2 || (ctx->scan_dir == 0 && sh.scan_at_end));
+        if (reverse) { fa.flags |= FZ_FLAG_REVERSE; ctx->rev_launches.fetch_add(1, std::memory_order_relaxed); }
+        if (!sp.partial) sh.scan_at_end = !reverse;
         const bool verify_follows = with_verify && !fa.fused;
         fa.host_hdr = (direct && !verify_follows && g0 + nblk >= G) ? reinterpret_cast<uint64_t>(d.cur().h_stage_dev) : 0;
         const bool ragged = geom_is_ragged(sh.geom);
@@ -1296,7 +1330,7 @@
     return fail(FZ_EDEVICE, "all-gather capacity kept overflowing");
 }
 
-int search_enqueue(fz_ctx *ctx, fz_seq *seq, const Search &q, bool with_verify, bool behind = false) {
+int search_enqueue(fz_ctx *ctx, fz_seq *seq, const Search &q, bool with_verify, bool behind = false, bool forward = false) {
     ctx->view = nullptr;
     ctx->view_n = 0;
     ctx->rows_ready = false;
@@ -1304,8 +1338,8 @@
     ctx->stats.bytes_scanned = ctx->stats.ngram_hits = ctx->stats.raw_matches = 0;
     ctx->stats.filter_ms = ctx->stats.verify_ms = ctx->stats.device_ms = 0;
     ctx->tref.clear();
-    int rc = for_each_shard(ctx, seq, [ctx, seq, &q, with_verify, behind](size_t si) {
-        return enqueue_shard(ctx, seq->shards[si], q, with_verify, true, behind);
+    int rc = for_each_shard(ctx, seq, [ctx, seq, &q, with_verify, behind, forward](size_t si) {
+        return enqueue_shard(ctx, seq->shards[si], q, with_verify, true, behind, forward);
     });
     if (rc) return rc;
     for (const Shard &sh : seq->shards) {
@@ -1380,7 +1414,7 @@
             }
             return FZ_OK;
         }
-        rc = search_enqueue(ctx, seq, q, with_verify);
+        rc = search_enqueue(ctx, seq, q, with_verify, false, true);
         if (rc) return rc;
     }
     return fail(FZ_EDEVICE, "result buffers kept overflowing");
@@ -1462,7 +1496,7 @@
                 d.dedup_zeroed = false;
                 d.gen_dedup_arg = reinterpret_cast<uint64_t>(d.d_gen_dedup);
             }
-            int rc = enqueue_shard(ctx, sh, q, false, false);
+            int rc = enqueue_shard(ctx, sh, q, false, false, false, attempt > 0);
             if (rc) return rc;
             SearchRun &run = d.cur().run;
             run.dedup_used = dedup;
@@ -5163,6 +5197,26 @@
     return FZ_OK;
 }
 
+int fz_debug_scan_walk(uint64_t ntiles, uint32_t grid, uint32_t n_regions, const uint64_t *table, uint32_t wg, uint32_t iter,
+                       int reversed, uint64_t *tile) {
+    if (!tile || (n_regions && !table) || n_regions > FZ_MAX_REGIONS || grid == 0 || wg >= grid) return fail(FZ_EINVAL, "bad argument");
+    uint32_t wg0[FZ_MAX_REGIONS] = {0}, nwg[FZ_MAX_REGIONS] = {0};
+    uint64_t tile0[FZ_MAX_REGIONS] = {0}, end[FZ_MAX_REGIONS] = {0};
+    for (uint32_t r = 0; r < n_regions; ++r) {
+        wg0[r] = (uint32_t)table[4 * r]; nwg[r] = (uint32_t)table[4 * r + 1]; tile0[r] = table[4 * r + 2]; end[r] = table[4 * r + 3];
+    }
+    *tile = fz_walk_tile(fz_scan_walk(n_regions, wg0, nwg, tile0, end, grid, ntiles, wg, reversed != 0), iter);
+    return FZ_OK;
+}
+
+int fz_debug_scan_direction(fz_ctx *ctx, fz_seq *seq, int *next_reversed, uint64_t *reversed_launches) {
+    if (!ctx || !next_reversed || !reversed_launches) return fail(FZ_EINVAL, "null argument");
+    const bool at_end = seq && !seq->shards.empty() && seq->shards[0].scan_at_end;
+    *next_reversed = (ctx->scan_dir == 2 || (ctx->scan_dir == 0 && at_end)) ? 1 : 0;
+    *reversed_launches = ctx->rev_launches.load(std::memory_order_relaxed);
+    return FZ_OK;
+}
+
 int fz_debug_scan_instance(uint32_t mode, const uint8_t *p, uint32_t m, uint32_t k, uint64_t buf_len, uint32_t n_cus,
                            uint32_t *n_launches, uint32_t *lean_mask, uint32_t *form) {
     if (!p || !n_launches || !lean_mask || !form || m == 0 || m / (k + 1) == 0 || n_cus == 0 || (mode != FZ_MODE_LEV && mode != FZ_MODE_SUBS))
@@ -5621,7 +5675,7 @@
     if (st->mode != FZ_MODE_GENERIC) {
         memset(&ctx->stats, 0, sizeof ctx->stats); ctx->tref.clear();
         ctx->stats.n_devices = 1;
-        rc = search_enqueue(ctx, st->seq, st->q, st->mode != FZ_MODE_EXACT);
+        rc = search_enqueue(ctx, st->seq, st->q, st->mode != FZ_MODE_EXACT, false, true);
         if (rc) return rc;
     }
     st->inflight = true;
@@ -6390,6 +6444,13 @@
     return FZ_OK;
 }
 
+int fz_set_scan_direction(fz_ctx *ctx, int mode) {
+    if (!ctx || mode < 0 || mode > 2) return fail(FZ_EINVAL, "scan direction must be 0 (alternate), 1 (forward) or 2 (reversed)");
+    if (ctx->npend || ctx->stream_inflight) return fail(FZ_EINVAL, "a search of this context is in flight");
+    ctx->scan_dir = mode;
+    return FZ_OK;
+}
+
 int fz_set_streams(fz_ctx *ctx, int n) {
     if (!ctx || (n != 1 && n != 2)) return fail(FZ_EINVAL, "streams must be 1 or 2");
     if (ctx->npend || ctx->stream_inflight) return fail(FZ_EINVAL, "a search of this context is in flight");
diff --git a/include/fzhip.h b/include/fzhip.h
--- a/include/fzhip.h
+++ b/include/fzhip.h
@@ -291,6 +291,11 @@
 int fz_debug_scan_instance(uint32_t mode, const uint8_t *p, uint32_t m, uint32_t k, uint64_t buf_len, uint32_t n_cus,
                            uint32_t *n_launches, uint32_t *lean_mask, uint32_t *form);
 
+int fz_debug_scan_walk(uint64_t ntiles, uint32_t grid, uint32_t n_regions, const uint64_t *table, uint32_t wg, uint32_t iter,
+                       int reversed, uint64_t *tile);
+
+int fz_debug_scan_direction(fz_ctx *ctx, fz_seq *seq, int *next_reversed, uint64_t *reversed_launches);
+
 int fz_debug_gather_merge(const void *blocks, uint32_t world, uint64_t cap, const uint64_t *own_lo, uint32_t L, fz_match **out,
                           uint64_t *n_out, uint64_t *need_cap);
 
@@ -298,6 +303,7 @@
 int  fz_mem_info(fz_ctx *ctx, uint64_t *free_bytes, uint64_t *total_bytes);
 int  fz_set_timing(fz_ctx *ctx, int on);
 int  fz_set_streams(fz_ctx *ctx, int n);
+int  fz_set_scan_direction(fz_ctx *ctx, int mode);
 int  fz_device_ms(fz_ctx *ctx, double *filter_ms, int cap);
 void fz_free(void *p);
 
```

Result: faster. 5722, median of 6 (+4.2%).
